# kcroker/Gadget-2.0.7-ngravs

Measured on AMD Instinct MI355X. Metric: particle-steps/s (tree+PM), higher is better.
Workload: dtype f64

## Files before the change

gadget-2.0.7-ngravs_amd/csrc/capi.hip:

```cpp
#include "engine.hpp"
#include "../../include/ngravs_peano.h"
#include <chrono>
#include <cmath>

static thread_local std::string g_create_error;

void ngravs_report(ngravs_ctx *ctx, int code, const std::string &msg)
{
  if(ctx)
    ctx->last_error = msg;
  else
    g_create_error = msg;
  if(ctx && ctx->on_fatal)
    ctx->on_fatal(code, msg.c_str());
  else
    fprintf(stderr, "task %d: endrun called with an error level of %d (%s)\n", ctx ? ctx->cfg.rank : 0, code, msg.c_str());
}

__global__ void k_pack_strided_f64(const unsigned char *src, long long stride, int ncomp, long long n, double *dst)
{
  long long i = blockIdx.x * (long long)blockDim.x + threadIdx.x;
  if(i >= n)
    return;
  const double *s = reinterpret_cast<const double *>(src + i * stride);
// ... 51 lines not shown
{
  long long k = blockIdx.x * (long long)blockDim.x + threadIdx.x;
  if(k >= count)
    return;
  const long long i = first + k;
  if(act[i] & 1)
    cost[idx[i]] = (double)nint[i];
}
__global__ void k_fill_f64(double *p, long long n, double v)
{
  long long i = blockIdx.x * (long long)blockDim.x + threadIdx.x;
  if(i < n)
    p[i] = v;
}
__global__ void k_fill_u8(unsigned char *p, long long n, unsigned char v)
{
  long long i = blockIdx.x * (long long)blockDim.x + threadIdx.x;
  if(i < n)
    p[i] = v;
}
__global__ void k_unpermute_f64(const unsigned int *idx, long long n, int ncomp, const double *src, double *dst)
{
  long long i = blockIdx.x * (long long)blockDim.x + threadIdx.x;
  if(i >= n)
    return;
  long long j = idx[i];
  for(int k = 0; k < ncomp; k++)
    dst[j * ncomp + k] = src[i * ncomp + k];
}
__global__ void k_unpermute_i2f(const unsigned int *idx, long long n, const int *src, float *dst)
{
  long long i = blockIdx.x * (long long)blockDim.x + threadIdx.x;
  if(i < n)
    dst[idx[i]] = (float)src[i];
}
__global__ void k_permute_f64(const unsigned int *idx, long long n, int ncomp, const double *src, double *dst)
{
  long long i = blockIdx.x * (long long)blockDim.x + threadIdx.x;
  if(i >= n)
    return;
  long long j = idx[i];
  for(int k = 0; k < ncomp; k++)
    dst[i * ncomp + k] = src[j * ncomp + k];
}
__global__ void k_permute_f64_lim(const unsigned int *idx, long long n, long long lim, int ncomp, const double *src, double *dst)
{
  long long i = blockIdx.x * (long long)blockDim.x + threadIdx.x;
  if(i >= n)
    return;
  long long j = idx[i];
  for(int k = 0; k < ncomp; k++)
    dst[i * ncomp + k] = j < lim ? src[j * ncomp + k] : 0.0;
}
__global__ void k_unpermute_f64_lim(const unsigned int *idx, long long n, long long lim, int ncomp, const double *src, double *dst)
{
  long long i = blockIdx.x * (long long)blockDim.x + threadIdx.x;
  if(i >= n)
    return;
  long long j = idx[i];
  if(j < lim)
    for(int k = 0; k < ncomp; k++)
      dst[j * ncomp + k] = src[i * ncomp + k];
}
__global__ void k_key18(const unsigned long long *k21, long long n, long long *out)
{
  long long i = blockIdx.x * (long long)blockDim.x + threadIdx.x;
  if(i < n)
    out[i] = (long long)(k21[i] >> (3 * (TREE_BITS - NGRAVS_BITS_PER_DIMENSION)));
}
__global__ void k_inverse_perm(const unsigned int *idx, long long n, int *inv)
{
  long long i = blockIdx.x * (long long)blockDim.x + threadIdx.x;
  if(i < n)
    inv[idx[i]] = (int)i;
}
__global__ void k_map_idx(const int *inv, const int *in, long long n, int *out)
{
  long long i = blockIdx.x * (long long)blockDim.x + threadIdx.x;
  if(i < n)
    out[i] = inv[in[i]];
}
#define GRID1(n) dim3((unsigned)(((n) + 255) / 256)), dim3(256)

extern "C" int ngravs_abi_version(void) { return NGRAVS_ABI_VERSION; }

extern "C" const char *ngravs_build_info(void)
{
  static char buf[512];
  snprintf(buf, sizeof(buf),
           "libngravs_hip abi=%d arch=gfx950 N_GRAVS<=%d NTAB=%d TREE_BITS=%d sizeof(config)=%zu sizeof(particles)=%zu "
           "sizeof(stats)=%zu walks=strict,group laws=none,newtonian,neg_newtonian,yukawa,coloyuk,bambam,sourcebambaryon,sourcebaryonbam",
           NGRAVS_ABI_VERSION, NGRAVS_MAX_GRAVS, NGRAVS_NTAB, NGRAVS_TREE_BITS, sizeof(ngravs_config_t),
           sizeof(ngravs_particles_t), sizeof(ngravs_stats_t));
  return buf;
}

extern "C" void ngravs_config_default(ngravs_config_t *cfg)
{
  memset(cfg, 0, sizeof(*cfg));
  cfg->abi_version = NGRAVS_ABI_VERSION;
  cfg->n_gravs = 1;
  cfg->G = 1.0;
  cfg->err_tol_theta = 0.5;
  cfg->err_tol_force_acc = 0.005;
  cfg->yukawa_imass = 60.0;
  cfg->tree_alloc_factor = 0.8;
  cfg->world_size = 1;
  for(int i = 0; i < NGRAVS_MAX_GRAVS; i++)
    for(int j = 0; j < NGRAVS_MAX_GRAVS; j++)
      {
        cfg->law_accel[i][j] = cfg->law_greens[i][j] = cfg->law_normed[i][j] = NGRAVS_LAW_NEWTON;
        cfg->law_spline[i][j] = NGRAVS_SPLINE_PLUMMER;
      }
}

static int check_config(const ngravs_config_t *cfg, std::string &why)
{
  if(cfg->abi_version != NGRAVS_ABI_VERSION)
    {
      why = "abi_version mismatch";
      return NGRAVS_ERR_ARG;
    }
  if(cfg->n_gravs < 1 || cfg->n_gravs > NGRAVS_MAX_GRAVS)
    {
      why = "n_gravs out of range";
      return NGRAVS_ERR_ARG;
    }
  if(cfg->pmgrid < 0 || (cfg->pmgrid & 1))
    {
      why = "PMGRID must be 0 (no mesh) or positive and even: the in-place real-to-complex mesh is laid out [N][N][N+2], which is the "
            "padding of the transform only for even N";
      return NGRAVS_ERR_ARG;
    }
  if(cfg->pmgrid && !cfg->periodic)
    {
      why = "non-periodic PM is disabled by ngravs itself (ngravs_core.c:235-242)";
      return NGRAVS_ERR_ARG;
    }
  if((cfg->periodic || cfg->pmgrid) && !(cfg->box_size > 0))
    {
      why = "box_size must be > 0";
      return NGRAVS_ERR_ARG;
    }
  if(cfg->pmgrid && cfg->type_to_grav[0] != 0)
    {
      why = "gas must be gravitational species 0 with PMGRID (ngravs_core.c:255-261)";
      return NGRAVS_ERR_WIRING;
    }
  if(cfg->world_size < 1 || cfg->rank < 0 || cfg->rank >= cfg->world_size)
    {
      why = "rank/world_size";
      return NGRAVS_ERR_ARG;
    }
  for(int t = 0; t < NGRAVS_NTYPES; t++)
    if(cfg->type_to_grav[t] < 0 || cfg->type_to_grav[t] >= cfg->n_gravs)
      {
        why = "TypeToGrav entry outside [0,N_GRAVS)";
        return NGRAVS_ERR_WIRING;
      }
  for(int i = 0; i < cfg->n_gravs; i++)
    for(int j = 0; j < cfg->n_gravs; j++)
      {
        auto bad = [](int id, int count) { return id < 0 || (id >= count && id < NGRAVS_LAW_USER0); };
        if(bad(cfg->law_accel[i][j], NGRAVS_LAW_COUNT) || bad(cfg->law_spline[i][j], NGRAVS_SPLINE_COUNT) ||
           bad(cfg->law_greens[i][j], NGRAVS_LAW_COUNT) || bad(cfg->law_normed[i][j], NGRAVS_LAW_COUNT))
          {
            why = "force-law table slot not wired (ngravs_core.c:321-360)";
            return NGRAVS_ERR_WIRING;
          }
        auto same = [](int a, int b, int p, int q) {
          return a == b || (a == p && b == q) || (a == q && b == p) || a >= NGRAVS_LAW_USER0 || b >= NGRAVS_LAW_USER0;
        };
        if(!same(cfg->law_accel[i][j], cfg->law_accel[j][i], NGRAVS_LAW_SOURCEBAM, NGRAVS_LAW_TARGETBAM) ||
           !same(cfg->law_spline[i][j], cfg->law_spline[j][i], NGRAVS_SPLINE_SOURCEBAM, NGRAVS_SPLINE_TARGETBAM) ||
           !same(cfg->law_normed[i][j], cfg->law_normed[j][i], -1, -1) || !same(cfg->law_greens[i][j], cfg->law_greens[j][i], -1, -1))
          {
            why = "force-law table violates Newton's third law (ngravs_core.c:371-403)";
            return NGRAVS_ERR_WIRING;
          }
      }
  if(cfg_has_bam(*cfg) && (cfg->pmgrid || cfg->periodic))
    {
      why = "the BAM laws have no Green's functions: tree-only, non-periodic runs (ngravs.c:189-194)";
      return NGRAVS_ERR_WIRING;
    }
  return NGRAVS_OK;
}

extern "C" int ngravs_create(const ngravs_config_t *cfg, ngravs_ctx **out) { return ngravs_create_with_laws(cfg, nullptr, 0, out); }

extern "C" int ngravs_create_with_laws(const ngravs_config_t *cfg, const ngravs_user_fn_t *fns, int nfns, ngravs_ctx **out)
{
  return ngravs_create_with_lattice(cfg, fns, nfns, nullptr, 0, out);
}

extern "C" int ngravs_create_with_lattice(const ngravs_config_t *cfg, const ngravs_user_fn_t *fns, int nfns,
                                          const ngravs_user_lattice_t *lat, int nlat, ngravs_ctx **out)
{
  if(!cfg || !out)
    return NGRAVS_ERR_ARG;
  *out = nullptr;
  std::string why;
  int rc = check_config(cfg, why);
  if(rc == NGRAVS_OK)
    rc = user_check_config(cfg, fns, nfns, lat, nlat, why);
  if(rc != NGRAVS_OK)
    {
      ngravs_report(nullptr, rc, why);
      return rc;
    }
  int ndev = 0;
  if(hipGetDeviceCount(&ndev) != hipSuccess || ndev <= 0)
    {
      ngravs_report(nullptr, NGRAVS_ERR_NO_DEVICE, "no HIP device: libngravs_hip has no CPU fallback");
      return NGRAVS_ERR_NO_DEVICE;
    }
  if(cfg->device < 0 || cfg->device >= ndev)
    return NGRAVS_ERR_ARG;
  ngravs_ctx *c = new ngravs_ctx;
  c->cfg = *cfg;
  c->user_fns.assign(fns, fns + nfns);
  c->user_lat.assign(lat, lat + nlat);
  memset(&c->stats, 0, sizeof(c->stats));
  if(hipSetDevice(cfg->device) != hipSuccess || hipStreamCreate(&c->stream) != hipSuccess ||
     hipEventCreate(&c->ev0) != hipSuccess || hipEventCreate(&c->ev1) != hipSuccess ||
     hipEventCreate(&c->evk0) != hipSuccess || hipEventCreate(&c->evk1) != hipSuccess || hipEventCreate(&c->ev_fork) != hipSuccess ||
     hipEventCreate(&c->ev_pm0) != hipSuccess || hipEventCreate(&c->ev_pm1) != hipSuccess || hipEventCreate(&c->ev_walk) != hipSuccess)
    {
      delete c;
      return NGRAVS_ERR_NO_DEVICE;
    }
  if(cfg->pmgrid)
    {
      c->asmth = cfg_asmth(cfg);
      c->rcut = cfg_rcut(cfg);
    }
  *out = c;
  return NGRAVS_OK;
}

extern "C" void ngravs_destroy(ngravs_ctx *c)
{
  if(!c)
    return;
  (void)hipSetDevice(c->cfg.device);
  (void)hipStreamSynchronize(c->stream);
  pm_release(c);
  pmslab_release(c);
  c->in_cost.release();
  c->in_pos.release();
  c->in_mass.release();
  c->in_oldacc.release();
  c->in_gsoft.release();
  c->gsoft_stage.release();
  c->s_soft.release();
  c->n_maxsoft.release();
  c->in_type.release();
  c->in_active.release();
  c->in_key.release();
  c->in_rec.release();
  c->in_id.release();
  c->dd_mask.release();
  c->dd_counts.release();
  c->dd_send.release();
  c->dd_recv.release();
  c->top.child.release();
  c->top.leaf.release();
  c->top.gcnt.release();
  c->top.info.release();
  c->top.gsum.release();
  c->top.leaf_owner.release();
  c->top.reqmask.release();
  c->top.leaf_sums.release();
  ngravs_host_toptree_free(&c->top.h);
  c->n_top.release();
  c->s_pm.release();
  c->s_type.release();
  c->s_active.release();
  c->s_oldacc.release();
  c->s_key.release();
  c->s_idx.release();
  c->idx_iota.release();
  c->sort_tmp.release();
  c->red_tmp.release();
  c->n_first.release();
  c->n_count.release();
  c->n_child.release();
  c->n_flags.release();
  c->n_nchild.release();
  c->n_geo.release();
  c->n_mom.release();
  c->n_npart.release();
  c->user_tab.release();
  c->user_green.release();
  c->scan_out.release();
  c->tb_count.release();
  c->scan_tmp.release();
  c->d_counters.release();
  c->d_levels.release();
  c->table.release();
  c->lat.release();
  c->walk_stack.release();
  c->walk_counters.release();
  c->walk_ovf.release();
  c->walk_tlist.release();
  c->walk_tmp.release();
  c->lvl_table.release();
  c->r_acc.release();
  c->r_pm.release();
  c->r_oldacc.release();
  c->r_nint.release();
  c->pm_rho.release();
  c->pm_phi.release();
  c->pm_force.release();
  c->pm_orig.release();
  c->out_tmp.release();
  c->out_tmpf.release();
  c->sph_vel_in.release();
  c->sph_h_in.release();
  c->sph_vel.release();
  c->sph_tlist.release();
  c->sph_tmp.release();
  c->sph_res.release();
  c->sph_row.release();
  c->sph_rounds.release();
  c->sph_counters.release();
  c->sph_col_in.release();
  c->sph_ts_in.release();
  c->sph_hsrc.release();
  c->sph_hmax.release();
  c->sph_gas_in.release();
  c->sph_ti_in.release();
  c->sph_tpos.release();
  c->sph_gmass.release();
  c->sph_gcount.release();
  c->sph_tg_in.release();
  c->sph_tg_ts.release();
  c->sph_tg_key.release();
  c->sph_tg_ord.release();
  c->sph_tg_res.release();
  (void)hipEventDestroy(c->ev0);
  (void)hipEventDestroy(c->ev1);
  (void)hipEventDestroy(c->evk0);
  (void)hipEventDestroy(c->evk1);
  for(hipEvent_t e : c->ev_batch)
    (void)hipEventDestroy(e);
  (void)hipEventDestroy(c->ev_fork);
  (void)hipEventDestroy(c->ev_pm0);
  (void)hipEventDestroy(c->ev_pm1);
  (void)hipEventDestroy(c->ev_walk);
  if(c->pm_stream)
    {
      (void)hipStreamSynchronize(c->pm_stream);
      (void)hipStreamSynchronize(c->walk_stream);
      (void)hipStreamDestroy(c->pm_stream);
      (void)hipStreamDestroy(c->walk_stream);
    }
  c->probe_out.release();
  (void)hipStreamDestroy(c->stream);
  delete c;
}

extern "C" void ngravs_set_fatal_handler(ngravs_ctx *ctx, ngravs_fatal_fn fn)
{
  if(ctx)
    ctx->on_fatal = fn;
}

extern "C" int ngravs_set_opening(ngravs_ctx *c, double theta, double errtol)
{
  if(!c)
    return NGRAVS_ERR_ARG;
  c->cfg.err_tol_theta = theta;
  c->cfg.err_tol_force_acc = errtol;
  return NGRAVS_OK;
}

extern "C" int ngravs_set_softening(ngravs_ctx *c, const double force_softening[NGRAVS_NTYPES])
{
  if(!c || !force_softening)
    return NGRAVS_ERR_ARG;
  for(int t = 0; t < NGRAVS_NTYPES; t++)
    if(!(force_softening[t] >= 0.0))
      {
        ngravs_report(c, NGRAVS_ERR_ARG, "ngravs_set_softening: negative or NaN softening length");
        return NGRAVS_ERR_ARG;
      }
  for(int t = 0; t < NGRAVS_NTYPES; t++)
    c->cfg.force_softening[t] = force_softening[t];
  c->gsoft_col_stale = c->gsoft_node_stale = true;
  return NGRAVS_OK;
}

extern "C" int ngravs_set_walk_mode(ngravs_ctx *c, int mode)
{
  if(!c || (mode != NGRAVS_WALK_STRICT && mode != NGRAVS_WALK_GROUP))
    return NGRAVS_ERR_ARG;
  c->cfg.walk_mode = mode;
  return NGRAVS_OK;
}

extern "C" int ngravs_get_config(ngravs_ctx *c, ngravs_config_t *out)
{
  if(!c || !out)
    return NGRAVS_ERR_ARG;
  *out = c->cfg;
  if(c->cfg.pmgrid)
    {
      out->asmth = c->asmth;
      out->rcut = c->rcut;
    }
  return NGRAVS_OK;
}

extern "C" int ngravs_set_tuning(ngravs_ctx *c, const char *name, double v)
{
  if(!c || !name)
    return NGRAVS_ERR_ARG;
  const std::string k(name);
  const long long iv = (long long)v;
  Tuning &t = c->tune;
  if(k == "walk_fused")
    t.walk_fused = iv != 0;
  else if(k == "walk_batch" && iv >= 0)
    t.walk_batch = iv;
  else if(k == "walk_waves" && iv >= 0 && iv <= 16)
    t.walk_waves = (int)iv;
  else if(k == "walk_lcap" && (iv == 0 || (iv >= 1024 && iv <= 65536)))
    {
      t.walk_lcap = (int)iv;
      c->walk_lcap = 0;
    }
  else if(k == "walk_root")
    t.walk_root = iv != 0;
  else if(k == "walk_compact")
    t.walk_compact = iv != 0;
  else if(k == "walk_spread" && iv >= 0 && iv <= 64 && (iv & (iv - 1)) == 0)
    t.walk_spread = (int)iv;
  else if(k == "walk_sg" && iv >= 0 && iv <= 16)
    t.walk_sg = (int)iv;
  else if(k == "walk_ring" && iv >= 0 && iv <= 1)
    t.walk_ring = (int)iv;
  else if(k == "walk_ring_k" && iv >= 0 && iv <= 8)
    t.walk_ring_k = (int)iv;
  else if(k == "walk_nleaf" && iv >= -1 && iv <= 8)
    t.walk_nleaf = (int)iv;
  else if(k == "walk_exact_reach")
    t.walk_exact_reach = iv != 0;
  else if(k == "sort_full")
    t.sort_full = iv != 0;
  else if(k == "tree_levelwise")
    t.tree_levelwise = iv != 0;
  else if(k == "dd_keep" && v >= 0 && v <= 0.25)
    t.dd_keep = v;
  else if(k == "pm_cus" && (iv == -1 || (iv >= 0 && iv <= 32 && iv % 8 == 0)))
    t.pm_cus = (int)iv;
  else if(k == "sph_verbose")
    t.sph_verbose = iv != 0;
  else
    {
      ngravs_report(c, NGRAVS_ERR_ARG, "ngravs_set_tuning: unknown name or value out of range: " + k);
      return NGRAVS_ERR_ARG;
    }
  return NGRAVS_OK;
}

extern "C" int ngravs_memcpy(ngravs_ctx *c, void *dst, const void *src, int64_t bytes, int kind)
{
  if(!c || bytes < 0 || kind < 1 || kind > 3 || (bytes > 0 && (!dst || !src)))
    return NGRAVS_ERR_ARG;
  if(bytes == 0)
    return NGRAVS_OK;
  (void)hipSetDevice(c->cfg.device);
  HIP_TRY(c, hipStreamSynchronize(c->stream));
  HIP_TRY(c, hipMemcpy(dst, src, (size_t)bytes, kind == 1 ? hipMemcpyHostToDevice : (kind == 2 ? hipMemcpyDeviceToHost : hipMemcpyDeviceToDevice)));
  return NGRAVS_OK;
}

extern "C" int ngravs_device_alloc(ngravs_ctx *c, void **ptr, int64_t bytes)
{
  if(!c || !ptr || bytes < 0)
    return NGRAVS_ERR_ARG;
  *ptr = nullptr;
  (void)hipSetDevice(c->cfg.device);
  if(hipMalloc(ptr, (size_t)(bytes > 0 ? bytes : 1)) != hipSuccess)
    return NGRAVS_ERR_NOMEM;
  return NGRAVS_OK;
}

extern "C" int ngravs_device_free(ngravs_ctx *c, void *ptr)
{
  if(!c)
    return NGRAVS_ERR_ARG;
  (void)hipSetDevice(c->cfg.device);
  if(ptr)
    (void)hipFree(ptr);
  return NGRAVS_OK;
}

static int upload_column_f64(ngravs_ctx *c, const void *src, int64_t stride, int ncomp, int64_t n, int on_device, double *dst)
{
  if(on_device)
    {
      if(stride == (int64_t)sizeof(double) * ncomp)
        HIP_TRY(c, hipMemcpyAsync(dst, src, sizeof(double) * ncomp * n, hipMemcpyDeviceToDevice, c->stream));
      else
        hipLaunchKernelGGL(k_pack_strided_f64, GRID1(n), 0, c->stream, (const unsigned char *)src, (long long)stride, ncomp,
                           (long long)n, dst);
      return NGRAVS_OK;
    }
  if(stride == (int64_t)sizeof(double) * ncomp)
    {
      HIP_TRY(c, hipMemcpyAsync(dst, src, sizeof(double) * ncomp * n, hipMemcpyHostToDevice, c->stream));
      HIP_TRY(c, hipStreamSynchronize(c->stream));
      return NGRAVS_OK;
    }
  c->host_stage.resize(sizeof(double) * ncomp * (size_t)n);
  double *h = reinterpret_cast<double *>(c->host_stage.data());
  for(int64_t i = 0; i < n; i++)
    memcpy(h + i * ncomp, (const unsigned char *)src + i * stride, sizeof(double) * ncomp);
  HIP_TRY(c, hipMemcpyAsync(dst, h, sizeof(double) * ncomp * n, hipMemcpyHostToDevice, c->stream));
  HIP_TRY(c, hipStreamSynchronize(c->stream));
  return NGRAVS_OK;
}

static double ev_ms(ngravs_ctx *c);

static int set_particles_impl(ngravs_ctx *c, const ngravs_particles_t *p, bool keep_tree)
{
  if(!c || !p || p->n < 0 || (p->n > 0 && (!p->pos || !p->mass || !p->type)))
    return NGRAVS_ERR_ARG;
  if(p->n == 0 && keep_tree)
    {
      if(!c->have_particles || c->n_local != 0)
        return NGRAVS_ERR_STATE;
      c->tree_stale = c->have_tree;
      return NGRAVS_OK;
    }
  if(p->n == 0)
    {
      (void)hipSetDevice(c->cfg.device);
      c->n = c->n_local = 0;
      c->own_order_nlocal = -1;
      c->sort_low = 35;
      c->all_active = true;
      c->walk_ia_ratio = 0;
      c->pm_solo_steps = 0, c->pm_auto_cus = -1;
      c->walk_unit_state = 4;
      c->have_particles = true;
      c->have_order = c->have_tree = c->have_pm = c->have_acc = false;
      c->gsoft_on = false;
      c->top.on = false;
      c->pm_parked = false;
      return NGRAVS_OK;
    }
  const bool keep_halo = keep_tree && c->n_local != c->n;
  if(keep_tree && (!c->have_order || !c->have_tree || p->n != c->n_local))
    {
      ngravs_report(c, NGRAVS_ERR_STATE, "ngravs_update_particles: needs a built tree over the same own particles");
      return NGRAVS_ERR_STATE;
    }
  if(p->n >= (1ll << 31) - 64)
    {
      ngravs_report(c, NGRAVS_ERR_ARG, "int particle indices (reference All.MaxPart is int): n must be < 2^31");
      return NGRAVS_ERR_ARG;
    }
  (void)hipSetDevice(c->cfg.device);
  const int64_t n = p->n;
  if(c->in_pos.ensure(3 * n) || c->in_mass.ensure(n) || c->in_oldacc.ensure(n) || c->in_type.ensure(n) || c->in_active.ensure(n) ||
     (!keep_tree && c->in_cost.ensure(n)))
    {
      ngravs_report(c, NGRAVS_ERR_NOMEM, "device allocation failed");
      return NGRAVS_ERR_NOMEM;
    }
  if(!keep_halo)
    c->n = n;
  c->n_local = n;
  if(!keep_tree)
    {
      if(c->own_order_nlocal != n)
        c->own_order_nlocal = -1;
      c->sort_low = 35;
    }
  int rc;
  if(!keep_tree && (rc = dd_fill_ids(c)))
    return rc;
  if((rc = upload_column_f64(c, p->pos, p->pos_stride, 3, n, p->on_device, c->in_pos.p)))
    return rc;
  if((rc = upload_column_f64(c, p->mass, p->mass_stride, 1, n, p->on_device, c->in_mass.p)))
    return rc;
  if(p->old_acc)
    {
      if((rc = upload_column_f64(c, p->old_acc, p->old_acc_stride, 1, n, p->on_device, c->in_oldacc.p)))
        return rc;
    }
  else
    hipLaunchKernelGGL(k_fill_f64, GRID1(n), 0, c->stream, c->in_oldacc.p, (long long)n, 0.0);
  if(!keep_tree)
    {
      if(p->grav_cost && p->on_device)
        hipLaunchKernelGGL(k_pack_strided_f32_to_f64, GRID1(n), 0, c->stream, (const unsigned char *)p->grav_cost,
                           (long long)p->grav_cost_stride, (long long)n, c->in_cost.p);
      else if(p->grav_cost)
        {
          c->host_stage.resize(sizeof(double) * (size_t)n);
          double *h = reinterpret_cast<double *>(c->host_stage.data());
// ... 240 lines not shown
      c->have_order = true;
      c->have_tree = c->tree_stale = c->have_pm = false;
      c->stats.t_domain = c->stats.t_peano = 0;
      return NGRAVS_OK;
    }
  HIP_TRY(c, hipEventRecord(c->ev0, c->stream));
  int rc = dom_find_extent(c);
  if(rc)
    return rc;
  HIP_TRY(c, hipEventRecord(c->ev1, c->stream));
  c->stats.t_domain = ev_ms(c) * 1e-3;
  HIP_TRY(c, hipEventRecord(c->ev0, c->stream));
  c->own_order_nlocal = -1;
  rc = dom_keys_and_sort(c);
  if(rc)
    return rc;
  c->own_order_nlocal = c->n_local;
  c->own_order_len = c->n;
  HIP_TRY(c, hipEventRecord(c->ev1, c->stream));
  c->stats.t_peano = ev_ms(c) * 1e-3;
  int64_t ws = c->cfg.world_size, r = c->cfg.rank;
  int64_t lo = (c->n * r) / ws, hi = (c->n * (r + 1)) / ws;
  lo = (lo / 64) * 64;
  hi = (r + 1 == ws) ? c->n : (hi / 64) * 64;
  c->shard_first = lo;
  c->shard_count = hi - lo;
  c->have_order = true;
  c->have_tree = false;
  c->gsoft_col_stale = c->gsoft_node_stale = true;
  c->tree_stale = false;
  if(c->have_pm)
    {
      if(c->r_pm.ensure(3 * c->n))
        return NGRAVS_ERR_NOMEM;
      hipLaunchKernelGGL(k_permute_f64_lim, GRID1(c->n), 0, c->stream, c->s_idx.p, (long long)c->n, (long long)c->n_local, 3, c->pm_orig.p,
                         c->r_pm.p);
      HIP_TRY(c, hipGetLastError());
    }
  return NGRAVS_OK;
}

extern "C" int ngravs_domain_decomposition(ngravs_ctx *c) { return domain_decomposition_impl(c, true); }

extern "C" int ngravs_discard_grav_pm(ngravs_ctx *c)
{
  if(!c)
    return NGRAVS_ERR_ARG;
  c->have_pm = false;
  c->pm_parked = false;
  return NGRAVS_OK;
}

extern "C" int64_t ngravs_force_treebuild(ngravs_ctx *c)
{
  if(!c || !c->have_order)
    return NGRAVS_ERR_STATE;
  (void)hipSetDevice(c->cfg.device);
  if(c->n == 0)
    {
      c->nnodes = 0;
      c->have_tree = true;
      c->tree_refit = false;
      c->stats.t_treebuild = 0;
      return 0;
    }
  if(hipEventRecord(c->ev0, c->stream) != hipSuccess)
    return NGRAVS_ERR_NO_DEVICE;
  int rc = tree_build(c);
  if(rc)
    return rc;
  if(hipEventRecord(c->ev1, c->stream) != hipSuccess)
    return NGRAVS_ERR_NO_DEVICE;
  c->stats.t_treebuild = ev_ms(c) * 1e-3;
  c->have_tree = true;
  c->tree_refit = false;
  c->gsoft_node_stale = true;
  return c->nnodes;
}

static int ensure_table(ngravs_ctx *c)
{
  if(!c->cfg.pmgrid || c->table_ready)
    return NGRAVS_OK;
  const int ng = c->cfg.n_gravs;
  std::vector<double> h((size_t)(ng * ng + 1) * NTAB);
  host_shortrange_table(&c->cfg, h.data(), nullptr, c->user_fns.data(), (int)c->user_fns.size());
  {
    WalkParams wp;
    make_walk_params(c, &wp);
    for(int t = 0; t < NTAB; t++)
      h[(size_t)ng * ng * NTAB + t] = exp(-wp.ym * (double)t * wp.inv_asmthfac);
  }
  if(c->table.ensure(h.size()))
    return NGRAVS_ERR_NOMEM;
  HIP_TRY(c, hipMemcpyAsync(c->table.p, h.data(), sizeof(double) * h.size(), hipMemcpyHostToDevice, c->stream));
  HIP_TRY(c, hipStreamSynchronize(c->stream));
  c->table_ready = true;
  return NGRAVS_OK;
}

static bool pm_cu_bit(int R, int b)
{
  const int x = b / 32, k = b - 33 * x;
  return b < 256 && k >= 0 && k % 8 == 0 && k / 8 < R / 8;
}

static int masked_streams(ngravs_ctx *c, int R)
{
  if(c->pm_stream && c->pm_stream_cus == R)
    return NGRAVS_OK;
  if(!c->device_cus)
    {
      hipDeviceProp_t prop;
      HIP_TRY(c, hipGetDeviceProperties(&prop, c->cfg.device));
      c->device_cus = prop.multiProcessorCount;
    }
  if(c->device_cus != 256 || R < 8 || R > 32 || R % 8)
    return NGRAVS_ERR_ARG;
  if(c->pm_stream)
    {
      HIP_TRY(c, hipStreamSynchronize(c->pm_stream));
      HIP_TRY(c, hipStreamSynchronize(c->walk_stream));
      (void)hipStreamDestroy(c->pm_stream);
      (void)hipStreamDestroy(c->walk_stream);
      c->pm_stream = c->walk_stream = nullptr;
      c->pm_stream_cus = 0;
    }
  uint32_t mp[8] = {0}, mw[8] = {0};
  for(int b = 0; b < 256; b++)
    (pm_cu_bit(R, b) ? mp : mw)[b / 32] |= 1u << (b % 32);
  hipStream_t sp = nullptr, sw = nullptr;
  if(hipExtStreamCreateWithCUMask(&sp, 8, mp) != hipSuccess || hipExtStreamCreateWithCUMask(&sw, 8, mw) != hipSuccess)
    {
      if(sp)
        (void)hipStreamDestroy(sp);
      (void)hipGetLastError();
      return NGRAVS_ERR_NO_DEVICE;
    }
  uint32_t gp[8] = {0}, gw[8] = {0};
  if(hipExtStreamGetCUMask(sp, 8, gp) != hipSuccess || hipExtStreamGetCUMask(sw, 8, gw) != hipSuccess || memcmp(gp, mp, sizeof mp) ||
     memcmp(gw, mw, sizeof mw))
    {
      (void)hipStreamDestroy(sp);
      (void)hipStreamDestroy(sw);
      (void)hipGetLastError();
      return NGRAVS_ERR_NO_DEVICE;
    }
  c->pm_stream = sp;
  c->walk_stream = sw;
  c->pm_stream_cus = R;
  return NGRAVS_OK;
}

static bool overlap_eligible(const ngravs_ctx *c)
{
  return c->cfg.pmgrid && c->cfg.periodic && c->cfg.world_size == 1 && !c->top.on && c->cfg.walk_mode == NGRAVS_WALK_GROUP &&
         c->n > 0 && c->n_local > 0;
}

static int gravity_tree_begin(ngravs_ctx *c, bool beside_pm, bool *masked, bool *empty)
{
  *masked = *empty = false;
  if(!c || !c->have_order)
    return NGRAVS_ERR_STATE;
  (void)hipSetDevice(c->cfg.device);
  int rc;
  if(!c->have_tree)
    {
      int64_t nn = ngravs_force_treebuild(c);
      if(nn < 0)
        return (int)nn;
    }
  else if(c->tree_stale && (rc = ngravs_force_update_tree(c)))
    return rc;
  if((rc = ensure_table(c)))
    return rc;
  if(c->n_local == 0)
    {
      c->stats.t_treewalk = 0;
      c->stats.walk_kernel_ms = 0;
      c->stats.interactions = 0;
      c->stats.n_active = 0;
      c->have_acc = true;
      *empty = true;
      return NGRAVS_OK;
    }
  HIP_TRY(c, hipEventRecord(c->ev0, c->stream));
  *masked = (beside_pm || (c->tune.pm_cus > 0 && overlap_eligible(c))) && masked_streams(c, beside_pm ? c->pm_stream_cus : c->tune.pm_cus) == NGRAVS_OK;
  if(*masked)
    {
      HIP_TRY(c, hipStreamWaitEvent(c->walk_stream, c->ev0, 0));
      OnStream on(c, c->walk_stream, c->device_cus - c->pm_stream_cus);
      return walk_enqueue(c);
    }
  return walk_enqueue(c);
}

static int gravity_tree_end(ngravs_ctx *c, bool masked, hipEvent_t pm_done)
{
  int rc;
  if(masked)
    {
      {
        OnStream on(c, c->walk_stream, c->device_cus - c->pm_stream_cus);
        if((rc = walk_complete(c)))
          return rc;
      }
      HIP_TRY(c, hipEventRecord(c->ev_walk, c->walk_stream));
      HIP_TRY(c, hipStreamWaitEvent(c->stream, c->ev_walk, 0));
    }
  else if((rc = walk_complete(c)))
    return rc;
  if(pm_done)
    HIP_TRY(c, hipStreamWaitEvent(c->stream, pm_done, 0));
  if((rc = walk_finish(c)))
    return rc;
  HIP_TRY(c, hipEventRecord(c->ev1, c->stream));
  c->stats.t_treewalk = ev_ms(c) * 1e-3;
  float kms = 0;
  (void)hipEventSynchronize(c->evk1);
  (void)hipEventElapsedTime(&kms, c->evk0, c->evk1);
  c->stats.walk_kernel_ms = kms;
  double h[2] = {0, 0};
  HIP_TRY(c, hipMemcpyAsync(h, c->red_tmp.p, 2 * sizeof(double), hipMemcpyDeviceToHost, c->stream));
  HIP_TRY(c, hipStreamSynchronize(c->stream));
  c->stats.interactions = h[0];
  c->stats.n_active = (int64_t)h[1];
  c->have_acc = true;
  if(c->cfg.pmgrid && c->cfg.walk_mode == NGRAVS_WALK_GROUP && h[1] > 0 && c->cfg.box_size > 0)
    {
      const double reach = (c->cfg.group_reach > 0 ? c->cfg.group_reach : NGRAVS_GROUP_REACH) * c->asmth;
      const double ntot = c->top.on && c->top.total_count > 0 ? c->top.total_count : (double)c->n;
      const double L = c->cfg.box_size, expect = 4.18879020478639 * reach * reach * reach * ntot / (L * L * L);
      const bool dense = c->walk_ntargets < 0 || c->walk_dense_tlist;
      if(expect > 0 && dense)
        {
          const double f_sg = c->walk_sg >= 4 ? 1.0 : (c->walk_sg >= 2 ? 1857.0 / 1393.0 : 1857.0 / 1079.0);
          const double f_s = c->walk_spread >= 2 ? 1079.0 / 871.0 : 1.0;
          c->walk_ia_ratio = (h[0] / h[1]) / expect * f_sg * f_s;
        }
    }
  if(c->shard_count > 0 && c->extent_override)
    hipLaunchKernelGGL(k_cost_update, GRID1(c->shard_count), 0, c->stream, c->s_idx.p, c->s_active.p, c->r_nint.p,
                       (long long)c->shard_first, (long long)c->shard_count, c->in_cost.p);
  return NGRAVS_OK;
}

extern "C" int ngravs_gravity_tree(ngravs_ctx *c)
{
  bool masked, empty;
  const int rc = gravity_tree_begin(c, false, &masked, &empty);
  return (rc || empty) ? rc : gravity_tree_end(c, masked, nullptr);
}

static int pm_on_masked_stream(ngravs_ctx *c)
{
  HIP_TRY(c, hipEventRecord(c->ev_fork, c->stream));
  HIP_TRY(c, hipStreamWaitEvent(c->pm_stream, c->ev_fork, 0));
  OnStream on(c, c->pm_stream, c->pm_stream_cus);
  HIP_TRY(c, hipEventRecord(c->ev_pm0, c->stream));
  int rc = pm_run(c);
  if(rc)
    return rc;
  HIP_TRY(c, hipEventRecord(c->ev_pm1, c->stream));
  return NGRAVS_OK;
}

extern "C" int ngravs_pmforce_periodic(ngravs_ctx *c)
{
  if(!c || !c->have_particles)
    return NGRAVS_ERR_STATE;
  (void)hipSetDevice(c->cfg.device);
  int rc;
  if(!c->have_order && (rc = ngravs_domain_decomposition(c)))
    return rc;
  if(!c->have_tree)
    {
      int64_t nn = ngravs_force_treebuild(c);
      if(nn < 0)
        return (int)nn;
    }
  else if(c->tree_stale && (rc = ngravs_force_update_tree(c)))
    return rc;
  if(c->tune.pm_cus > 0 && overlap_eligible(c) && masked_streams(c, c->tune.pm_cus) == NGRAVS_OK)
    {
      if((rc = pm_on_masked_stream(c)))
        return rc;
      float ms = 0;
      HIP_TRY(c, hipEventSynchronize(c->ev_pm1));
      (void)hipEventElapsedTime(&ms, c->ev_pm0, c->ev_pm1);
      HIP_TRY(c, hipStreamWaitEvent(c->stream, c->ev_pm1, 0));
      c->stats.t_pm = ms * 1e-3;
      return NGRAVS_OK;
    }
  HIP_TRY(c, hipEventRecord(c->ev0, c->stream));
  if((rc = pm_run(c)))
    return rc;
  HIP_TRY(c, hipEventRecord(c->ev1, c->stream));
  c->stats.t_pm = ev_ms(c) * 1e-3;
  return NGRAVS_OK;
}

static const double PM_CU_SCALE[4] = {17.75, 9.07, 6.16, 4.74};
static const double PM_FIT_MARGIN = 1.05, PM_SHARE_COST = 1.04;
static int choose_pm_cus(ngravs_ctx *c)
{
  if(!overlap_eligible(c))
    return 0;
  if(c->tune.pm_cus >= 0)
    return c->tune.pm_cus;
  if(c->pm_auto_cus >= 0)
    return c->pm_auto_cus;
  if(c->pm_solo_steps < 2 || c->pm_solo_ms <= 0 || c->walk_solo_ms <= 0)
    return 0;
  c->pm_auto_cus = 0;
  for(int m = 1; m <= 4; m++)
    {
      const double walk = c->walk_solo_ms * 256.0 / (256 - 8 * m);
      if(c->pm_solo_ms * PM_CU_SCALE[m - 1] * PM_FIT_MARGIN < walk)
        {
          if(walk * PM_SHARE_COST < 0.99 * (c->pm_solo_ms + c->walk_solo_ms))
            c->pm_auto_cus = 8 * m;
          break;
        }
    }
  return c->pm_auto_cus;
}

extern "C" int ngravs_compute_accelerations(ngravs_ctx *c, int pm_step)
{
  if(!c || !c->have_particles)
    return NGRAVS_ERR_STATE;
  int rc;
  if((rc = domain_decomposition_impl(c, !(pm_step && c->cfg.pmgrid))))
    return rc;
  c->last_pm_cus = 0;
  if(!(pm_step && c->cfg.pmgrid))
    return ngravs_gravity_tree(c);
  const int R = choose_pm_cus(c);
  if(R > 0 && masked_streams(c, R) == NGRAVS_OK)
    {
      int64_t nn = ngravs_force_treebuild(c);
      if(nn < 0)
        return (int)nn;
      bool masked, empty;
      if((rc = gravity_tree_begin(c, true, &masked, &empty)))
        return rc;
      if((rc = pm_on_masked_stream(c)))
        return rc;
      if(!empty && (rc = gravity_tree_end(c, masked, c->ev_pm1)))
        return rc;
      float ms = 0;
      (void)hipEventElapsedTime(&ms, c->ev_pm0, c->ev_pm1);
      c->stats.t_pm = ms * 1e-3;
      c->last_pm_cus = R;
      if(c->tune.pm_cus < 0 && ms > c->stats.walk_kernel_ms)
        c->pm_auto_cus = R < 32 ? R + 8 : 0;
      return NGRAVS_OK;
    }
  if((rc = ngravs_pmforce_periodic(c)))
    return rc;
  if((rc = ngravs_gravity_tree(c)))
    return rc;
  if(overlap_eligible(c) && c->tune.pm_cus < 0 && c->pm_auto_cus < 0)
    {
      c->pm_solo_ms = c->stats.t_pm * 1e3;
      c->walk_solo_ms = c->stats.walk_kernel_ms;
      c->pm_solo_steps++;
    }
  return NGRAVS_OK;
}

static int download_strided(ngravs_ctx *c, const void *dsrc, size_t elem, int ncomp, int64_t n, void *dst, int64_t stride,
                            int on_device)
{
  const size_t row = elem * ncomp;
  if(on_device)
    {
      if((size_t)stride != row)
        {
          ngravs_report(c, NGRAVS_ERR_ARG, "device outputs must be contiguous");
          return NGRAVS_ERR_ARG;
        }
      HIP_TRY(c, hipMemcpyAsync(dst, dsrc, row * n, hipMemcpyDeviceToDevice, c->stream));
      HIP_TRY(c, hipStreamSynchronize(c->stream));
      return NGRAVS_OK;
    }
  if((size_t)stride == row)
    {
      HIP_TRY(c, hipMemcpyAsync(dst, dsrc, row * n, hipMemcpyDeviceToHost, c->stream));
      HIP_TRY(c, hipStreamSynchronize(c->stream));
      return NGRAVS_OK;
    }
  c->host_stage.resize(row * (size_t)n);
  HIP_TRY(c, hipMemcpyAsync(c->host_stage.data(), dsrc, row * n, hipMemcpyDeviceToHost, c->stream));
  HIP_TRY(c, hipStreamSynchronize(c->stream));
  for(int64_t i = 0; i < n; i++)
    memcpy((unsigned char *)dst + i * stride, c->host_stage.data() + i * row, row);
  return NGRAVS_OK;
}

static int deliver(ngravs_ctx *c, const void *dsrc, size_t elem, int ncomp, int64_t n, void *dst, int64_t stride, int on_device,
                   const unsigned char *d_mask)
{
  if(!d_mask)
    return download_strided(c, dsrc, elem, ncomp, n, dst, stride, on_device);
  const size_t row = elem * ncomp;
  if(on_device)
    {
      if((size_t)stride != row)
        {
          ngravs_report(c, NGRAVS_ERR_ARG, "device outputs must be contiguous");
          return NGRAVS_ERR_ARG;
        }
      if(elem == sizeof(double))
        hipLaunchKernelGGL(k_copy_masked_f64, GRID1(n), 0, c->stream, d_mask, (long long)n, ncomp, (const double *)dsrc, (double *)dst);
      else
        hipLaunchKernelGGL(k_copy_masked_f32, GRID1(n), 0, c->stream, d_mask, (long long)n, (const float *)dsrc, (float *)dst);
      HIP_TRY(c, hipStreamSynchronize(c->stream));
      return NGRAVS_OK;
    }
  c->host_stage.resize(row * (size_t)n + (size_t)n);
  unsigned char *hm = c->host_stage.data() + row * (size_t)n;
  HIP_TRY(c, hipMemcpyAsync(c->host_stage.data(), dsrc, row * n, hipMemcpyDeviceToHost, c->stream));
  HIP_TRY(c, hipMemcpyAsync(hm, d_mask, (size_t)n, hipMemcpyDeviceToHost, c->stream));
  HIP_TRY(c, hipStreamSynchronize(c->stream));
  for(int64_t i = 0; i < n; i++)
    if(hm[i] & 1)
      memcpy((unsigned char *)dst + i * stride, c->host_stage.data() + i * row, row);
  return NGRAVS_OK;
}

extern "C" int ngravs_get_accel(ngravs_ctx *c, double *grav_accel, int64_t accel_stride, double *grav_pm, int64_t pm_stride,
                                double *old_acc, int64_t old_acc_stride, float *grav_cost, int64_t cost_stride, int on_device,
                                int only_active)
{
  if(!c || !c->have_order)
    return NGRAVS_ERR_STATE;
  (void)hipSetDevice(c->cfg.device);
  const int64_t n = c->n, nl = c->n_local;
  if(nl == 0)
    return NGRAVS_OK;
  if(c->out_tmp.ensure(3 * n) || c->out_tmpf.ensure(n))
    return NGRAVS_ERR_NOMEM;
  const unsigned char *mask = only_active ? c->in_active.p : nullptr;
  int rc;
  if(grav_accel)
    {
      if(!c->have_acc)
        return NGRAVS_ERR_STATE;
      HIP_TRY(c, hipMemsetAsync(c->out_tmp.p, 0, sizeof(double) * 3 * n, c->stream));
      hipLaunchKernelGGL(k_unpermute_f64, GRID1(n), 0, c->stream, c->s_idx.p, (long long)n, 3, c->r_acc.p, c->out_tmp.p);
      if((rc = deliver(c, c->out_tmp.p, sizeof(double), 3, nl, grav_accel, accel_stride, on_device, mask)))
        return rc;
    }
  if(grav_pm)
    {
      if(!c->have_pm)
        return NGRAVS_ERR_STATE;
      hipLaunchKernelGGL(k_unpermute_f64, GRID1(n), 0, c->stream, c->s_idx.p, (long long)n, 3, c->r_pm.p, c->out_tmp.p);
      if((rc = deliver(c, c->out_tmp.p, sizeof(double), 3, nl, grav_pm, pm_stride, on_device, nullptr)))
        return rc;
    }
  if(old_acc)
    {
      if(!c->have_acc)
        return NGRAVS_ERR_STATE;
      hipLaunchKernelGGL(k_unpermute_f64, GRID1(n), 0, c->stream, c->s_idx.p, (long long)n, 1, c->r_oldacc.p, c->out_tmp.p);
      if((rc = deliver(c, c->out_tmp.p, sizeof(double), 1, nl, old_acc, old_acc_stride, on_device, mask)))
        return rc;
    }
  if(grav_cost)
    {
      if(!c->have_acc)
        return NGRAVS_ERR_STATE;
      hipLaunchKernelGGL(k_unpermute_i2f, GRID1(n), 0, c->stream, c->s_idx.p, (long long)n, c->r_nint.p, c->out_tmpf.p);
      if((rc = deliver(c, c->out_tmpf.p, sizeof(float), 1, nl, grav_cost, cost_stride, on_device, mask)))
        return rc;
    }
  return NGRAVS_OK;
}

extern "C" int ngravs_get_stats(ngravs_ctx *c, ngravs_stats_t *out)
{
  if(!c || !out)
    return NGRAVS_ERR_ARG;
  *out = c->stats;
  return NGRAVS_OK;
}

static std::string kept_state(const ngravs_ctx *c, const char *who)
{
  char b[320];
  snprintf(b, sizeof(b), "%s: no kept decomposition to work on (own rows %lld, rows at the cut %lld, working set %lld, tree %d, top %d, task %d of %d)", who,
           (long long)c->n_local, (long long)c->top.own_leaf_n, (long long)c->n, (int)c->have_tree, (int)c->top.on, c->top.kept_rank, c->top.kept_world);
  return std::string(b);
}
extern "C" int ngravs_dd_leaf_sums_kept(ngravs_ctx *c, void **dev_sums, int64_t *count)
{
  if(!c || !dev_sums || !count)
    return NGRAVS_ERR_ARG;
  (void)hipSetDevice(c->cfg.device);
  const int rc = dd_leaf_sums_kept(c, dev_sums, count);
  if(rc == NGRAVS_ERR_STATE)
    ngravs_report(c, rc, kept_state(c, "ngravs_dd_leaf_sums_kept"));
  return rc;
}
extern "C" int ngravs_dd_pack_leaves_kept(ngravs_ctx *c, int64_t *counts, void **dev_records, int64_t *nrec)
{
  if(!c || !counts || !dev_records || !nrec)
    return NGRAVS_ERR_ARG;
  (void)hipSetDevice(c->cfg.device);
  const int rc = dd_pack_leaves_kept(c, counts, dev_records, nrec);
  if(rc == NGRAVS_ERR_STATE)
    ngravs_report(c, rc, kept_state(c, "ngravs_dd_pack_leaves_kept"));
  return rc;
}
extern "C" int ngravs_dd_refresh_halo(ngravs_ctx *c, const void *dev_records, int64_t nrec)
{
  if(!c || nrec < 0 || (nrec > 0 && !dev_records))
    return NGRAVS_ERR_ARG;
  (void)hipSetDevice(c->cfg.device);
  const int rc = dd_refresh_halo(c, dev_records, nrec);
  if(rc == NGRAVS_ERR_STATE)
    ngravs_report(c, rc, kept_state(c, "ngravs_dd_refresh_halo"));
  return rc;
}
extern "C" int ngravs_dd_update_top(ngravs_ctx *c, const double *node_sums, const double *leaf_len)
{
  if(!c)
    return NGRAVS_ERR_ARG;
  (void)hipSetDevice(c->cfg.device);
  const int rc = dd_update_top(c, node_sums, leaf_len);
  if(rc == NGRAVS_ERR_STATE)
    ngravs_report(c, rc, kept_state(c, "ngravs_dd_update_top"));
  return rc;
}
extern "C" int ngravs_dd_get_kept(ngravs_ctx *c, int32_t *rank, int32_t *world, const int32_t **leaf_owner, const uint8_t **present,
                                  const double **node_sums)
{
  if(!c)
    return NGRAVS_ERR_ARG;
  const TopTree &t = c->top;
  if(!(t.on && t.h.nnode > 0 && t.own_leaf_n == c->n_local && t.kept_rank >= 0 && (int)t.h_leaf_owner.size() == t.h.nleaf &&
       (int)t.h_present.size() == t.h.nleaf))
    {
      ngravs_report(c, NGRAVS_ERR_STATE, kept_state(c, "ngravs_dd_get_kept"));
      return NGRAVS_ERR_STATE;
    }
  if(rank)
    *rank = t.kept_rank;
  if(world)
    *world = t.kept_world;
  if(leaf_owner)
    *leaf_owner = t.h_leaf_owner.data();
  if(present)
    *present = t.h_present.data();
  if(node_sums)
    *node_sums = t.h_node_sums.data();
  return NGRAVS_OK;
}

extern "C" int ngravs_walk_unopened(ngravs_ctx *c, int64_t *count)
{
  if(!c || !count)
    return NGRAVS_ERR_ARG;
  *count = (int64_t)c->walk_unopened;
  return NGRAVS_OK;
}

extern "C" int ngravs_get_domain(ngravs_ctx *c, double out[8])
{
  if(!c || !c->have_order)
    return NGRAVS_ERR_STATE;
  memcpy(out, c->dom, sizeof(double) * 8);
  return NGRAVS_OK;
}

extern "C" int ngravs_get_keys(ngravs_ctx *c, int64_t *keys, int on_device)
{
  if(!c || !c->have_order || !keys)
    return NGRAVS_ERR_STATE;
  (void)hipSetDevice(c->cfg.device);
  const int64_t n = c->n;
  if(c->out_tmp.ensure(3 * n))
    return NGRAVS_ERR_NOMEM;
  long long *tmp = reinterpret_cast<long long *>(c->out_tmp.p);
  hipLaunchKernelGGL(k_key18, GRID1(n), 0, c->stream, c->in_key.p, (long long)n, tmp);
  return download_strided(c, tmp, sizeof(long long), 1, c->n_local, keys, sizeof(long long), on_device);
}

extern "C" int ngravs_get_order(ngravs_ctx *c, int32_t *order, int on_device)
{
  if(!c || !c->have_order || !order)
    return NGRAVS_ERR_STATE;
  (void)hipSetDevice(c->cfg.device);
  return download_strided(c, c->s_idx.p, sizeof(int), 1, c->n, order, sizeof(int), on_device);
}

extern "C" int ngravs_get_shard(ngravs_ctx *c, int64_t *first, int64_t *count)
{
  if(!c || !c->have_order)
    return NGRAVS_ERR_STATE;
  if(first)
    *first = c->shard_first;
  if(count)
    *count = c->shard_count;
// ... 959 lines not shown
```

gadget-2.0.7-ngravs_amd/csrc/engine.hpp:

```cpp
#pragma once
#include <hip/hip_runtime.h>
#include <cstdint>
#include <cstdio>
#include <cstdlib>
#include <cstring>
#include <string>
#include <utility>
#include <vector>
#include "../../include/ngravs_host.h"

#define NG_MAX NGRAVS_MAX_GRAVS
#define NTAB NGRAVS_NTAB
#define TREE_BITS NGRAVS_TREE_BITS
#define FLAG_BUCKET 64
#define FLAG_PSEUDO 128
#define FLAG_PARTIAL 256
#define FLAG_SPECIES_SHIFT 9
#define FLAG_SPECIES_SLOTS 8
#define FLAG_SPECIES_MASK (0xffff << FLAG_SPECIES_SHIFT)
#define MAX_LEVELS (TREE_BITS + 1)

struct ngravs_ctx;

#define HIP_TRY(ctx, expr)                                                                        \
  do                                                                                              \
    {                                                                                             \
      hipError_t e__ = (expr);                                                                    \
      if(e__ != hipSuccess)                                                                       \
        {                                                                                         \
          ngravs_report(ctx, NGRAVS_ERR_NO_DEVICE, std::string(#expr) + ": " + hipGetErrorString(e__)); \
          return NGRAVS_ERR_NO_DEVICE;                                                            \
        }                                                                                         \
    }                                                                                             \
  while(0)

void ngravs_report(ngravs_ctx *ctx, int code, const std::string &msg);

template <typename T> struct DevBuf
{
  T *p = nullptr;
  size_t cap = 0;
  int ensure(size_t n)
  {
    if(n <= cap)
      return 0;
    if(p)
      (void)hipFree(p);
    p = nullptr;
    cap = 0;
    size_t want = n + n / 16 + 64;
    if(hipMalloc((void **)&p, want * sizeof(T)) != hipSuccess)
      return -1;
    cap = want;
    return 0;
  }
  void release()
  {
    if(p)
      (void)hipFree(p);
    p = nullptr;
    cap = 0;
  }
};

#define UL_NC 8
struct UserTabs
{
  const double *coef, *spl;
  int e_lo, n_oct, S;
  int nh, Ss;
  double h[NGRAVS_NTYPES];
};
__host__ __device__ inline double ul_poly(const double *c, double t)
{
  double v = c[7];
  for(int j = 6; j >= 0; j--)
    v = v * t + c[j];
  return v;
}
__host__ __device__ inline double ul_g(const UserTabs &u, int k, double r)
{
  int e;
  (void)frexp(r, &e);
  int o = e - u.e_lo;
  const double m = ldexp(r, -(u.e_lo + (o < 0 ? 0 : (o >= u.n_oct ? u.n_oct - 1 : o))));
  double s = (m - 0.5) * (2 * u.S);
  s = o < 0 ? 0.0 : (o >= u.n_oct ? (double)u.S : s);
  o = o < 0 ? 0 : (o >= u.n_oct ? u.n_oct - 1 : o);
  s = s >= 0 ? (s <= u.S ? s : (double)u.S) : 0.0;
  int j = (int)s;
  j = j >= u.S ? u.S - 1 : j;
  return ul_poly(u.coef + ((size_t)(k * u.n_oct + o) * u.S + j) * UL_NC, 2 * (s - j) - 1);
}
__host__ __device__ inline double ul_spline(const UserTabs &u, int k, double h, double r)
{
  if(u.nh == 0)
    return 0.0;
  int i = 0;
  for(int q = 1; q < u.nh; q++)
    if(fabs(u.h[q] - h) < fabs(u.h[i] - h))
      i = q;
  double s = r / h * u.Ss;
  s = s >= 0 ? (s <= u.Ss ? s : (double)u.Ss) : 0.0;
  int j = (int)s;
  j = j >= u.Ss ? u.Ss - 1 : j;
  return ul_poly(u.spl + ((size_t)(k * u.nh + i) * u.Ss + j) * UL_NC, 2 * (s - j) - 1);
}

struct WalkParams
{
  int ng, periodic, pm, use_theta;
  int nleaf;
  int exact_reach;
  double box, boxhalf;
  double theta2;
  double errtol_acc;
  double rcut, rcut2, asmthfac, utor2wpi, reach2;
  double ym;
  double bam_eps;
  double fac_intp;
  double fsoft[NGRAVS_NTYPES];
  int t2g[NGRAVS_NTYPES];
  unsigned t2g_packed;
  double cN[NG_MAX][NG_MAX], cY[NG_MAX][NG_MAX], cS[NG_MAX][NG_MAX];
  int ntab_lds;
  int tab_slot[NG_MAX * NG_MAX];
  int slot_src[NG_MAX * NG_MAX];
  int exp_tab;
  double inv_asmthfac;
  double ec[4];
  int src_in_box;
  int bam;
  int law_accel[NG_MAX][NG_MAX], law_spline[NG_MAX][NG_MAX];
  int user;
  UserTabs ut;
};

struct TreeView
{
  const int *first, *count, *child, *flags;
  const int *npart;
  const double4 *geo, *mom;
  int nnodes;
  const int *ltab;
  int ltab_level;
  double ltab_corner[3], ltab_cl;
  const double *soft;
  const double *maxsoft;
};

struct Tuning
{
  int walk_fused = 0, walk_waves = 0, walk_lcap = 0, walk_root = 0, walk_compact = 1, walk_spread = 0, walk_exact_reach = 0, walk_sg = 0, walk_nleaf = -1;
  long long walk_batch = 0;
  int sort_full = 0;
  int tree_levelwise = 0;
  double dd_keep = 0;
  int walk_ring = 1;
  int walk_ring_k = 0;
  int pm_cus = -1;
  int sph_verbose = 0;
};

#define TOP_CW(ng) (7 + 4 * (ng))
struct TopTree
{
  double total_count = 0;
  bool on = false;
  double import_reach = 0;
  ngravs_toptree h = {0, 0, 0, 0, nullptr, nullptr, nullptr, nullptr, nullptr};
  DevBuf<int> child, leaf;
  DevBuf<int> gcnt;
  DevBuf<unsigned char> info;
  DevBuf<double> gsum;
  DevBuf<int> leaf_owner;
  DevBuf<unsigned long long> reqmask;
  DevBuf<double> leaf_sums;
  DevBuf<int> own_leaf;
  long long own_leaf_n = -1;
  int kept_rank = -1, kept_world = 0;
  std::vector<int> h_leaf_owner;
  std::vector<unsigned char> h_present;
  std::vector<double> h_node_sums;
  DevBuf<int> kept_row;
  std::vector<int64_t> kept_counts;
  long long kept_total = -1;
  DevBuf<double> kept_sums;
  DevBuf<double> leaf_len;
};

struct PmSlab
{
  int world = 0, rank = 0, N = 0, stage = -1;
  int xs = 0, nx = 0, ys = 0, ny = 0;
  int lo[3] = {0, 0, 0}, ext[3] = {0, 0, 0};
  int elo[3] = {0, 0, 0}, eext[3] = {0, 0, 0};
  std::vector<int> bbox;
  std::vector<int64_t> scount, rcount;
  long long edesc_off = 0;
  DevBuf<double> brick, slab, tbuf, ebrick, fmesh, send, recv;
  DevBuf<long long> desc;
  std::vector<long long> hdesc[2];
  int hdesc_turn = 0;
  void *plan2f = nullptr, *plan2i = nullptr, *plan1 = nullptr;
  int plan_N = 0, plan_nx = 0, plan_ny = 0;
  double bytes_sent[4] = {0, 0, 0, 0};
};

struct ngravs_ctx
{
  ngravs_config_t cfg;
  Tuning tune;
  PmSlab pms;
  TopTree top;
  DevBuf<int> n_top;
  ngravs_fatal_fn on_fatal = nullptr;
  hipStream_t stream = nullptr;
  double asmth = 0, rcut = 0;
  int64_t n = 0;
  int64_t n_local = 0;
  bool extent_override = false;
  double ext_lo[3], ext_hi[3];
  int dd_last_what = -1;
  long long dd_last_sent = 0;
  bool have_particles = false, have_order = false, have_tree = false, have_pm = false, have_acc = false;
  bool pm_parked = false;
  double dom[8] = {0, 0, 0, 0, 0, 0, 0, 0};
  double pos_lo[3] = {0, 0, 0}, pos_hi[3] = {-1, -1, -1};
  int64_t shard_first = 0, shard_count = 0;

  DevBuf<double> in_pos, in_mass, in_oldacc;
  DevBuf<double> in_cost;
  DevBuf<int> in_type;
  DevBuf<unsigned char> in_active;
  DevBuf<double2> in_rec;
  DevBuf<unsigned long long> in_key;
  DevBuf<long long> in_id;
  DevBuf<unsigned long long> dd_mask, dd_counts;
  int sort_low = 35;
  long long own_order_nlocal = -1, own_order_len = 0;
  DevBuf<unsigned char> dd_send, dd_recv;
  DevBuf<double4> s_pm;
  DevBuf<unsigned char> s_type, s_active;
  DevBuf<double> s_oldacc;
  DevBuf<unsigned long long> s_key;
  DevBuf<unsigned int> s_idx, idx_iota;
  DevBuf<unsigned char> sort_tmp;
  DevBuf<double> red_tmp;
  int64_t max_nodes = 0, nnodes = 0;
  bool tree_refit = false;
  bool tree_stale = false;
  int nlevels = 0;
  DevBuf<int> lvl_table;
  int lvl_table_level = 0;
  int64_t level_start[MAX_LEVELS + 2];
  DevBuf<int> n_first, n_count, n_child, n_flags, n_nchild;
  DevBuf<double4> n_geo, n_mom;
  DevBuf<int> tb_count;
  DevBuf<int> n_npart;
  DevBuf<int> scan_out;
  DevBuf<unsigned char> scan_tmp;
  DevBuf<int> d_counters;
  DevBuf<int> d_levels;
  long long level_hint[MAX_LEVELS + 2] = {0};
  DevBuf<double> table;
  bool table_ready = false;
  DevBuf<double> lat;
  bool lat_ready = false;
  DevBuf<int> walk_stack;
  DevBuf<int> walk_tlist;
  DevBuf<unsigned char> walk_tmp;
  long long walk_ntargets = -1;
  bool walk_dense_tlist = false;
  int walk_spread = 0;
  int walk_sg = 1;
  long long walk_unopened = 0;
  int walk_unit_state = 4;
  double walk_ia_ratio = 0;
  bool all_active = true;
  DevBuf<int> walk_ovf;
  DevBuf<int> walk_counters;
  DevBuf<double> r_acc, r_pm, r_oldacc;
  DevBuf<int> r_nint;
  int pm_plan_n = 0;
  void *fft_fwd = nullptr, *fft_inv = nullptr;
  DevBuf<double> pm_rho;
  DevBuf<double> pm_force;
  DevBuf<double> pm_phi;
  DevBuf<double> pm_orig;
  DevBuf<double> out_tmp;
  DevBuf<float> out_tmpf;
  std::vector<unsigned char> host_stage;
  ngravs_stats_t stats;
  hipEvent_t ev0 = nullptr, ev1 = nullptr, evk0 = nullptr, evk1 = nullptr;
  std::vector<hipEvent_t> ev_batch;
  int walk_batches = 0;
  int walk_lcap = 0;
  int walk_scap = 0;
  bool walk_used_split = false;
  long long walk_cap_n = -1;
  size_t walk_cap_stack = 0;
  size_t walk_cap_bytes = 0;
  std::vector<std::pair<const void *, size_t>> walk_lds_set;
  std::string last_error;
  std::vector<ngravs_user_fn_t> user_fns;
  std::vector<ngravs_user_lattice_t> user_lat;
  DevBuf<double> user_tab;
  UserTabs user_ut = {};
  bool user_ready = false;
  double user_soft[NGRAVS_NTYPES] = {0, 0, 0, 0, 0, 0};
  int last_walk_kernel = 0;
  bool gsoft_on = false;
  bool gsoft_col_stale = true, gsoft_node_stale = true;
  DevBuf<double> in_gsoft;
  DevBuf<double> gsoft_stage;
  DevBuf<double> s_soft;
  DevBuf<double> n_maxsoft;
  hipStream_t pm_stream = nullptr, walk_stream = nullptr;
  int pm_stream_cus = 0;
  int device_cus = 0;
  int stream_cus = 0;
  int last_pm_cus = 0;
  double pm_solo_ms = 0, walk_solo_ms = 0;
  int pm_solo_steps = 0;
  int pm_auto_cus = -1;
  hipEvent_t ev_fork = nullptr, ev_pm0 = nullptr, ev_pm1 = nullptr, ev_walk = nullptr;
  DevBuf<int> probe_out;
  DevBuf<double> user_green;
  long long user_green_nk2 = 0;
  DevBuf<double> sph_vel_in, sph_h_in;
  DevBuf<double> sph_vel;
  DevBuf<int> sph_tlist;
  DevBuf<unsigned char> sph_tmp;
  DevBuf<double> sph_res;
  DevBuf<int> sph_row, sph_rounds;
  DevBuf<unsigned long long> sph_counters;
  DevBuf<double> sph_col_in;
  DevBuf<int> sph_ts_in;
  DevBuf<double> sph_hsrc;
  DevBuf<double> sph_hmax;
  DevBuf<double> sph_gas_in;
  DevBuf<int> sph_ti_in;
  DevBuf<int> sph_tpos;
  DevBuf<double> sph_gmass;
  DevBuf<int> sph_gcount;
  DevBuf<double> sph_tg_in;
  DevBuf<int> sph_tg_ts;
  DevBuf<unsigned long long> sph_tg_key;
  DevBuf<unsigned int> sph_tg_ord;
  DevBuf<double> sph_tg_res;
};

struct OnStream
{
  ngravs_ctx *c;
  hipStream_t s0;
  int n0;
  OnStream(ngravs_ctx *c_, hipStream_t s, int cus) : c(c_), s0(c_->stream), n0(c_->stream_cus)
  {
    c->stream = s;
    c->stream_cus = cus;
  }
  ~OnStream()
  {
    c->stream = s0;
    c->stream_cus = n0;
  }
};

int dom_find_extent(ngravs_ctx *c);
int dom_keys_and_sort(ngravs_ctx *c);
int dom_keys_only(ngravs_ctx *c, const double *d_pos, int64_t n, const double corner[3], double fac, int bits,
                  long long *d_keys);
int dd_local_extent(ngravs_ctx *c, double lo[3], double hi[3]);
void dd_apply_extent(ngravs_ctx *c, const double lo[3], const double hi[3]);
int dd_set_toptree(ngravs_ctx *c, int nnode, const int *child);
int dd_leaf_sums(ngravs_ctx *c, void **dev_sums, int64_t *count);
int dd_pack(ngravs_ctx *c, int what, const int *leaf_owner, int nranks, int me, int64_t *counts, void **dev_records, int64_t *nrec);
int dd_apply_migration(ngravs_ctx *c, const void *dev_records, int64_t nrec);
int dd_get_dest(ngravs_ctx *c, const int *leaf_owner, int *dest);
int dd_target_bounds(ngravs_ctx *c, double out[2]);
int dd_pack_leaves(ngravs_ctx *c, const unsigned long long *reqmask, int nranks, int me, int64_t *counts, void **dev_records, int64_t *nrec);
int dd_set_top(ngravs_ctx *c, const double *node_sums, const unsigned char *present);
int dd_set_halo(ngravs_ctx *c, const void *dev_records, int64_t nrec);
int dd_leaf_sums_kept(ngravs_ctx *c, void **dev_sums, int64_t *count);
int dd_pack_leaves_kept(ngravs_ctx *c, int64_t *counts, void **dev_records, int64_t *nrec);
int dd_refresh_halo(ngravs_ctx *c, const void *dev_records, int64_t nrec);
int dd_update_top(ngravs_ctx *c, const double *node_sums, const double *leaf_len);
int dd_peano_order_own(ngravs_ctx *c, int force);
int dd_fill_ids(ngravs_ctx *c);
int dd_record_doubles(const ngravs_ctx *c, int what);
int tree_build(ngravs_ctx *c);
int tree_moments(ngravs_ctx *c, bool refit, bool counts = false);
int tree_top_leaf_len(ngravs_ctx *c, double *dev_kept_sums, int stride);
int tree_top_refit(ngravs_ctx *c);
int dom_regather(ngravs_ctx *c);
static inline bool cfg_has_bam(const ngravs_config_t &cfg)
{
  for(int i = 0; i < cfg.n_gravs; i++)
    for(int j = 0; j < cfg.n_gravs; j++)
      if((cfg.law_accel[i][j] >= NGRAVS_LAW_BAMBAM && cfg.law_accel[i][j] < NGRAVS_LAW_USER0) ||
         (cfg.law_spline[i][j] >= NGRAVS_SPLINE_BAMBAM && cfg.law_spline[i][j] < NGRAVS_SPLINE_USER0))
        return true;
  return false;
}
static inline bool cfg_has_user(const ngravs_config_t &cfg)
{
  for(int i = 0; i < cfg.n_gravs; i++)
    for(int j = 0; j < cfg.n_gravs; j++)
      if(cfg.law_accel[i][j] >= NGRAVS_LAW_USER0 || cfg.law_spline[i][j] >= NGRAVS_SPLINE_USER0)
        return true;
  return false;
}
int user_check_config(const ngravs_config_t *cfg, const ngravs_user_fn_t *fns, int nfns, const ngravs_user_lattice_t *lat, int nlat,
                      std::string &why);
ngravs_lattice_fn user_lattice_fn(const ngravs_ctx *c, int a, int b);
bool user_lattice_complete(const ngravs_ctx *c);
int user_lattice_tabulate(ngravs_lattice_fn fn, double box, double *out, std::string &why);
void ngravs_report(ngravs_ctx *ctx, int code, const std::string &msg);
int user_tables_ensure(ngravs_ctx *c, double r_need);
int user_green_ensure(ngravs_ctx *c);
double user_normed(const ngravs_user_fn_t *fns, int nfns, int law, double k2);
void make_walk_params(const ngravs_ctx *c, WalkParams *wp);
int walk_run(ngravs_ctx *c);
int walk_enqueue(ngravs_ctx *c);
int walk_complete(ngravs_ctx *c);
int walk_finish(ngravs_ctx *c);
int direct_run(ngravs_ctx *c, const int *d_idx, int64_t nt, double *d_acc);
int direct_run_targets(ngravs_ctx *c, const double4 *d_tpm, const int *d_ttype, int64_t nt, double *d_acc, double r_need = 0);
int adaptive_refresh(ngravs_ctx *c, bool nodes);
int eval_ring_slots(const WalkParams &wp, bool yuk, int waves);
int launch_eval_ring(ngravs_ctx *c, const TreeView &tv, const WalkParams &wp, bool yuk, int nblk, int waves, int K, const int *region,
                     const int *gcount, long long g0, long long nb, int lcap, int scap, int S, const int *tlist, int SG, long long t_count);
#define SPH_KC1 2.546479089470
#define SPH_KC2 15.278874536822
#define SPH_KC3 45.836623610466
#define SPH_KC4 30.557749073644
#define SPH_KC5 5.092958178941
#define SPH_KC6 (-15.278874536822)
#define SPH_NORM_COEFF 4.188790204786
#define SPH_MAXITER 150
__host__ __device__ inline void sph_spline(double u, double hinv3, double hinv4, double *wk, double *dwk)
{
  if(u < 0.5)
    {
      *wk = hinv3 * (SPH_KC1 + SPH_KC2 * (u - 1) * u * u);
      *dwk = hinv4 * u * (SPH_KC3 * u - SPH_KC4);
    }
  else
    {
      *wk = hinv3 * SPH_KC5 * (1.0 - u) * (1.0 - u) * (1.0 - u);
      *dwk = hinv4 * SPH_KC6 * (1.0 - u) * (1.0 - u);
    }
}
enum { SPH_HSML = 0, SPH_DENSITY, SPH_NUMNGB, SPH_DIVVEL, SPH_CURLVEL, SPH_DHSML, SPH_NRES };
struct SphStats
{
  long long targets, bad_hsml, failed, stack_ovf, max_rounds, sum_rounds, candidates, neighbours;
};
int sph_density_run(ngravs_ctx *c, double des_num_ngb, double max_dev, double min_hsml, SphStats *st);
int sph_hsml_guess_run(ngravs_ctx *c, double des_num_ngb, int only_unset, long long *rows, long long *bad_mass);
enum { SPH_HS_VX = 0, SPH_HS_VY, SPH_HS_VZ, SPH_HS_H, SPH_HS_RHO, SPH_HS_POR2, SPH_HS_CSJ, SPH_HS_F2, SPH_HS_TS, SPH_HS_CSI, SPH_HS_F1,
       SPH_HS_NCOL };
enum { SPH_HY_ACCX = 0, SPH_HY_ACCY, SPH_HY_ACCZ, SPH_HY_DTENTR, SPH_HY_MAXSIG, SPH_HY_NRES };
struct SphHydroParams
{
  int periodic, comoving, limiter, have_ts;
  double box, boxhalf;
  double hubble_a2, fac_mu, fac_vsic_fix;
  double visc, tbi, gamma;
};
struct SphHydroStats
{
  long long targets, bad_hsml, bad_density, bad_pressure, stack_ovf, candidates, pairs;
};
int sph_hydro_run(ngravs_ctx *c, const SphHydroParams &hp, SphHydroStats *st);
enum { SPH_GAS_PRESSURE = SPH_NRES, SPH_GAS_HYDRO, SPH_GAS_NRES = SPH_GAS_HYDRO + SPH_HY_NRES };
struct SphGasParams
{
  double des, dev, minh;
  int ti_current, have_dte;
};
int sph_gas_run(ngravs_ctx *c, const SphGasParams &gp, const SphHydroParams &hp, SphStats *ds, SphHydroStats *hs, hipEvent_t ev_density,
                hipEvent_t ev_prep);
struct SphScatterCols
{
  unsigned char *dst[SPH_GAS_NRES];
  long long stride[SPH_GAS_NRES];
};
int sph_scatter_cols(ngravs_ctx *c, long long nt, const SphScatterCols &cols);
int sph_scatter(ngravs_ctx *c, const double *src, long long nt, double *dst, long long stride);
enum { SPH_SUM_RHO = 0, SPH_SUM_NGB, SPH_SUM_DHR, SPH_SUM_DIV, SPH_SUM_ROTX, SPH_SUM_ROTY, SPH_SUM_ROTZ, SPH_NSUMS };
enum { SPH_TG_H = 6, SPH_TG_MASS, SPH_TG_RHO, SPH_TG_P, SPH_TG_DHSML, SPH_TG_F1, SPH_TG_NCOL };
struct SphSumsStats
{
  long long bad_hsml, bad_density, bad_pressure, bad_pos, stack_ovf, candidates, pairs;
};
int sph_density_sums_run(ngravs_ctx *c, long long nt, SphSumsStats *st);
int sph_hydro_sums_run(ngravs_ctx *c, const SphHydroParams &hp, long long nt, int have_tts, SphSumsStats *st, SphHydroStats *own);
__host__ __device__ inline int sph_density_update_one(const double *s, double des, double dev, double minh, double *h_io, double *left_io,
                                                      double *right_io, int *rounds_io, double *out6)
{
#pragma clang fp contract(off)
  double h = *h_io, left = *left_io, right = *right_io;
  const int nr = ++*rounds_io;
  const double numngb = s[SPH_SUM_NGB], rho = s[SPH_SUM_RHO];
  const double dhf = 1 / (1 + h * s[SPH_SUM_DHR] / (3 * rho));
  bool redo = numngb < (des - dev) || (numngb > (des + dev) && h > 1.01 * minh);
  if(redo && left > 0 && right > 0 && (right - left) < 1.0e-3 * left)
    redo = false;
  if(!redo)
    {
      out6[SPH_HSML] = h;
      out6[SPH_DENSITY] = rho;
      out6[SPH_NUMNGB] = numngb;
      out6[SPH_DIVVEL] = s[SPH_SUM_DIV] / rho;
      out6[SPH_CURLVEL] = sqrt(s[SPH_SUM_ROTX] * s[SPH_SUM_ROTX] + s[SPH_SUM_ROTY] * s[SPH_SUM_ROTY] + s[SPH_SUM_ROTZ] * s[SPH_SUM_ROTZ]) / rho;
      out6[SPH_DHSML] = dhf;
      return 0;
    }
  if(numngb < (des - dev))
    left = fmax(h, left);
  else if(right != 0)
    {
      if(h < right)
        right = h;
    }
  else
    right = h;
  if(right > 0 && left > 0)
    h = pow(0.5 * (pow(left, 3) + pow(right, 3)), 1.0 / 3);
  else
    {
      const bool newton = fabs(numngb - des) < 0.5 * des;
      const double fac = 1 - (numngb - des) / (3 * numngb) * dhf;
      if(right == 0 && left > 0)
        h *= newton ? fac : 1.26;
      if(right > 0 && left == 0)
        h = newton ? h * fac : h / 1.26;
    }
  if(h < minh)
    h = minh;
  *h_io = h, *left_io = left, *right_io = right;
  return nr > SPH_MAXITER ? 2 : 1;
}
int sph_density_update_device(long long n, const double *sums, double *h, double *left, double *right, int *rounds, double des, double dev,
                              double minh, int *accepted, double *const out[SPH_NRES], long long *failed);
int pm_run(ngravs_ctx *c);
int pm_deposit(ngravs_ctx *c);
int pm_finish(ngravs_ctx *c);
void pm_release(ngravs_ctx *c);
int pmslab_begin(ngravs_ctx *c, int rank, int world, int bbox[6]);
int pmslab_pack(ngravs_ctx *c, int stage, const int *all_bbox, int64_t *send_counts, int64_t *recv_counts, void **send, void **recv);
int pmslab_unpack(ngravs_ctx *c, int stage);
void pmslab_release(ngravs_ctx *c);
void host_shortrange_table(const ngravs_config_t *cfg, double *force, double *pot, const ngravs_user_fn_t *fns = nullptr, int nfns = 0);
double cfg_asmth(const ngravs_config_t *c);
double cfg_rcut(const ngravs_config_t *c);
```

gadget-2.0.7-ngravs_amd/csrc/eval_asm.inc:

```


#define ER_FST_OFF_ET "16640"
#define ER_FST_OFF_NOET "256"

#define ER_YUK_ET \
  "v_fract_f64_e32 v[118:119], v[118:119]\n"                                   \
  "v_mul_f64 v[122:123], v[118:119], %[ec3]\n" \
  "v_lshl_add_u32 v113, v112, 3, %[etab]\n" \
  "v_add_f64 v[122:123], v[122:123], -%[ec2]\n" \
  "ds_read_b64 v[124:125], v113\n"                                             \
  "v_lshl_add_u32 v112, v112, 3, %[trow]\n" \
  "v_fma_f64 v[122:123], v[122:123], v[118:119], %[ec1]\n" \
  "ds_read_b64 v[112:113], v112\n"                                             \
  "v_fma_f64 v[122:123], v[122:123], v[118:119], -%[ec0]\n" \
  "v_mul_f64 v[120:121], v[114:115], v[114:115]\n"                             \
  "v_fma_f64 v[122:123], v[122:123], v[118:119], 1.0\n"                        \
  "s_waitcnt lgkmcnt(1)\n" \
  "v_mul_f64 v[122:123], v[124:125], v[122:123]\n"                             \
  "v_mul_f64 v[122:123], %[cY], v[122:123]\n" \
  "v_fma_f64 v[124:125], %[ym], v[114:115], v[120:121]\n"                      \
  "v_mul_f64 v[122:123], v[124:125], v[122:123]\n" \
  "v_fmac_f64_e32 v[122:123], %[cN], v[120:121]\n"

#define ER_NOYUK \
  "v_lshl_add_u32 v112, v112, 3, %[trow]\n" \
  "ds_read_b64 v[112:113], v112\n" \
  "v_mul_f64 v[120:121], v[114:115], v[114:115]\n" \
  "v_mul_f64 v[122:123], %[cN], v[120:121]\n"

#define ER_DIRECT_ASM \
  "s_mov_b32 s89, 0\n" \
  "ds_read_b128 v[104:107], %[ptr]\n" \
  "ds_read_b128 v[108:111], %[ptr] offset:16\n" \
  "s_bitcmp1_b32 %[n], 0\n"                                                    \
  "s_cbranch_scc0 L_ed_pairs_%=\n" \
  "s_waitcnt lgkmcnt(0)\n" \
  "v_add_f64 v[104:105], v[104:105], -%[tpx]\n" \
  "v_add_f64 v[106:107], v[106:107], -%[tpy]\n" \
  "v_mul_f64 v[112:113], v[106:107], v[106:107]\n" \
  "v_add_f64 v[108:109], v[108:109], -%[tpz]\n" \
  "v_fmac_f64_e32 v[112:113], v[104:105], v[104:105]\n" \
  "v_fmac_f64_e32 v[112:113], v[108:109], v[108:109]\n" \
  "v_add_f64 v[116:117], v[112:113], %[tiny]\n"                                \
  "v_rsq_f64_e32 v[114:115], v[116:117]\n" \
  "v_cmp_gt_f64_e32 vcc, %[h2max], v[112:113]\n"                               \
  "v_mul_f64 v[118:119], v[116:117], v[114:115]\n"                             \
  "v_fma_f64 v[118:119], -v[118:119], v[114:115], 1.0\n" \
  "v_mul_f64 v[120:121], v[114:115], 0.5\n" \
  "v_fma_f64 v[114:115], v[120:121], v[118:119], v[114:115]\n"                 \
  "v_mul_f64 v[120:121], v[114:115], v[114:115]\n" \
  "v_mul_f64 v[122:123], %[cN], v[120:121]\n"                                  \
  "v_mul_f64 v[122:123], v[110:111], v[122:123]\n" \
  "v_mul_f64 v[122:123], v[114:115], v[122:123]\n"                             \
  "s_cbranch_vccnz L_ed_softs_%=\n" \
  "L_ed_accs_%=:\n" \
  "v_fmac_f64_e32 %[ax], v[104:105], v[122:123]\n" \
  "v_fmac_f64_e32 %[ay], v[106:107], v[122:123]\n" \
  "v_fmac_f64_e32 %[az], v[108:109], v[122:123]\n" \
  "s_mov_b32 s89, 1\n" \
  "v_add_u32_e32 %[ptr], 32, %[ptr]\n" \
  "ds_read_b128 v[104:107], %[ptr]\n"                                          \
  "ds_read_b128 v[108:111], %[ptr] offset:16\n" \
  "L_ed_pairs_%=:\n" \
  "s_cmp_lt_u32 s89, %[n]\n" \
  "s_cbranch_scc0 L_ed_done_%=\n" \
  "L_ed_topx_%=:\n" \
  "s_waitcnt lgkmcnt(0)\n" \
  "ds_read_b128 v[96:99], %[ptr] offset:32\n" \
  "ds_read_b128 v[100:103], %[ptr] offset:48\n" \
  "v_add_f64 v[104:105], v[104:105], -%[tpx]\n" \
  "v_add_f64 v[106:107], v[106:107], -%[tpy]\n" \
  "v_mul_f64 v[112:113], v[106:107], v[106:107]\n" \
  "v_add_f64 v[108:109], v[108:109], -%[tpz]\n" \
  "v_fmac_f64_e32 v[112:113], v[104:105], v[104:105]\n" \
  "v_fmac_f64_e32 v[112:113], v[108:109], v[108:109]\n" \
  "v_add_f64 v[116:117], v[112:113], %[tiny]\n"                                \
  "v_rsq_f64_e32 v[114:115], v[116:117]\n" \
  "v_cmp_gt_f64_e32 vcc, %[h2max], v[112:113]\n"                               \
  "v_mul_f64 v[118:119], v[116:117], v[114:115]\n"                             \
  "v_fma_f64 v[118:119], -v[118:119], v[114:115], 1.0\n" \
  "v_mul_f64 v[120:121], v[114:115], 0.5\n" \
  "v_fma_f64 v[114:115], v[120:121], v[118:119], v[114:115]\n"                 \
  "v_mul_f64 v[120:121], v[114:115], v[114:115]\n" \
  "v_mul_f64 v[122:123], %[cN], v[120:121]\n"                                  \
  "v_mul_f64 v[122:123], v[110:111], v[122:123]\n" \
  "v_mul_f64 v[122:123], v[114:115], v[122:123]\n"                             \
  "s_cbranch_vccnz L_ed_softx_%=\n" \
  "L_ed_accx_%=:\n" \
  "v_fmac_f64_e32 %[ax], v[104:105], v[122:123]\n" \
  "v_fmac_f64_e32 %[ay], v[106:107], v[122:123]\n" \
  "v_fmac_f64_e32 %[az], v[108:109], v[122:123]\n" \
  "s_waitcnt lgkmcnt(0)\n" \
  "v_add_u32_e32 %[ptr], 64, %[ptr]\n" \
  "ds_read_b128 v[104:107], %[ptr]\n"                                          \
  "ds_read_b128 v[108:111], %[ptr] offset:16\n" \
  "v_add_f64 v[96:97], v[96:97], -%[tpx]\n" \
  "v_add_f64 v[98:99], v[98:99], -%[tpy]\n" \
  "v_mul_f64 v[112:113], v[98:99], v[98:99]\n" \
  "v_add_f64 v[100:101], v[100:101], -%[tpz]\n" \
  "v_fmac_f64_e32 v[112:113], v[96:97], v[96:97]\n" \
  "v_fmac_f64_e32 v[112:113], v[100:101], v[100:101]\n" \
  "v_add_f64 v[116:117], v[112:113], %[tiny]\n"                                \
  "v_rsq_f64_e32 v[114:115], v[116:117]\n" \
  "v_cmp_gt_f64_e32 vcc, %[h2max], v[112:113]\n"                               \
  "v_mul_f64 v[118:119], v[116:117], v[114:115]\n"                             \
  "v_fma_f64 v[118:119], -v[118:119], v[114:115], 1.0\n" \
  "v_mul_f64 v[120:121], v[114:115], 0.5\n" \
  "v_fma_f64 v[114:115], v[120:121], v[118:119], v[114:115]\n"                 \
  "v_mul_f64 v[120:121], v[114:115], v[114:115]\n" \
  "v_mul_f64 v[122:123], %[cN], v[120:121]\n"                                  \
  "v_mul_f64 v[122:123], v[102:103], v[122:123]\n" \
  "v_mul_f64 v[122:123], v[114:115], v[122:123]\n"                             \
  "s_cbranch_vccnz L_ed_softy_%=\n" \
  "L_ed_accy_%=:\n" \
  "v_fmac_f64_e32 %[ax], v[96:97], v[122:123]\n" \
  "v_fmac_f64_e32 %[ay], v[98:99], v[122:123]\n" \
  "v_fmac_f64_e32 %[az], v[100:101], v[122:123]\n" \
  "s_add_u32 s89, s89, 2\n" \
  "s_cmp_lt_u32 s89, %[n]\n" \
  "s_cbranch_scc1 L_ed_topx_%=\n" \
  "s_branch L_ed_done_%=\n" \
  "L_ed_softs_%=:\n" \
  "v_mul_f64 v[116:117], v[116:117], v[114:115]\n"                             \
  "v_add_u32_e32 v118, s89, %[tyb]\n"                                          \
  "ds_read_u8 v118, v118\n" \
  "s_waitcnt lgkmcnt(0)\n" \
  "v_lshl_add_u32 v118, v118, 3, %[fst]\n" \
  "ds_read_b64 v[124:125], v118\n"                                             \
  "s_waitcnt lgkmcnt(0)\n" \
  "v_max_f64 v[124:125], v[124:125], %[hT]\n"                                  \
  "v_rcp_f64_e32 v[112:113], v[124:125]\n" \
  "v_cmp_lt_f64_e64 s[94:95], v[116:117], v[124:125]\n"                        \
  "v_fma_f64 v[118:119], -v[124:125], v[112:113], 1.0\n"                       \
  "v_fma_f64 v[112:113], v[112:113], v[118:119], v[112:113]\n" \
  "v_fma_f64 v[118:119], -v[124:125], v[112:113], 1.0\n" \
  "v_fma_f64 v[112:113], v[112:113], v[118:119], v[112:113]\n"                 \
  "v_mul_f64 v[114:115], v[124:125], v[114:115]\n"                             \
  "v_mul_f64 v[118:119], v[116:117], v[112:113]\n"                             \
  "v_mul_f64 v[120:121], v[118:119], v[118:119]\n"                             \
  "v_ldexp_f64 v[124:125], v[118:119], 5\n"                                    \
  "s_mov_b32 s90, 0x33333333\n" \
  "s_mov_b32 s91, 0x40433333\n" \
  "v_add_f64 v[124:125], v[124:125], -s[90:91]\n" \
  "s_mov_b32 s92, 0x55555611\n" \
  "s_mov_b32 s93, 0x40255555\n" \
  "v_fma_f64 v[124:125], v[120:121], v[124:125], s[92:93]\n"                   \
  "v_mul_f64 v[116:117], v[120:121], v[118:119]\n"                             \
  "v_mul_f64 v[120:121], v[120:121], s[90:91]\n"                               \
  "s_mov_b32 s90, 0x555554f8\n" \
  "s_mov_b32 s91, 0x40355555\n" \
  "v_add_f64 v[120:121], v[120:121], s[90:91]\n"                               \
  "s_mov_b32 s90, 0x00000000\n" \
  "s_mov_b32 s91, 0xc0480000\n" \
  "v_fma_f64 v[120:121], v[118:119], s[90:91], v[120:121]\n"                   \
  "v_fma_f64 v[120:121], -v[116:117], s[92:93], v[120:121]\n"                  \
  "v_mul_f64 v[116:117], v[114:115], v[114:115]\n" \
  "v_mul_f64 v[116:117], v[116:117], v[114:115]\n"                             \
  "s_mov_b32 s90, 0x11116ee4\n" \
  "s_mov_b32 s91, 0x3fb11111\n" \
  "v_fma_f64 v[120:121], -v[116:117], s[90:91], v[120:121]\n"                  \
  "v_cmp_gt_f64_e32 vcc, 0.5, v[118:119]\n"                                    \
  "v_cndmask_b32_e32 v120, v120, v124, vcc\n" \
  "v_cndmask_b32_e32 v121, v121, v125, vcc\n" \
  "v_mul_f64 v[124:125], %[cS], v[110:111]\n"                                  \
  "v_mul_f64 v[124:125], v[124:125], v[112:113]\n" \
  "v_mul_f64 v[124:125], v[124:125], v[112:113]\n" \
  "v_mul_f64 v[124:125], v[124:125], v[112:113]\n" \
  "v_mul_f64 v[124:125], v[124:125], v[120:121]\n" \
  "v_cndmask_b32_e64 v122, v122, v124, s[94:95]\n" \
  "v_cndmask_b32_e64 v123, v123, v125, s[94:95]\n" \
  "s_branch L_ed_accs_%=\n" \
  "L_ed_softx_%=:\n" \
  "v_mul_f64 v[116:117], v[116:117], v[114:115]\n"                             \
  "v_add_u32_e32 v118, s89, %[tyb]\n"                                          \
  "ds_read_u8 v118, v118\n" \
  "s_waitcnt lgkmcnt(0)\n" \
  "v_lshl_add_u32 v118, v118, 3, %[fst]\n" \
  "ds_read_b64 v[124:125], v118\n"                                             \
  "s_waitcnt lgkmcnt(0)\n" \
  "v_max_f64 v[124:125], v[124:125], %[hT]\n"                                  \
  "v_rcp_f64_e32 v[112:113], v[124:125]\n" \
  "v_cmp_lt_f64_e64 s[94:95], v[116:117], v[124:125]\n"                        \
  "v_fma_f64 v[118:119], -v[124:125], v[112:113], 1.0\n"                       \
  "v_fma_f64 v[112:113], v[112:113], v[118:119], v[112:113]\n" \
  "v_fma_f64 v[118:119], -v[124:125], v[112:113], 1.0\n" \
  "v_fma_f64 v[112:113], v[112:113], v[118:119], v[112:113]\n"                 \
  "v_mul_f64 v[114:115], v[124:125], v[114:115]\n"                             \
  "v_mul_f64 v[118:119], v[116:117], v[112:113]\n"                             \
  "v_mul_f64 v[120:121], v[118:119], v[118:119]\n"                             \
  "v_ldexp_f64 v[124:125], v[118:119], 5\n"                                    \
  "s_mov_b32 s90, 0x33333333\n" \
  "s_mov_b32 s91, 0x40433333\n" \
  "v_add_f64 v[124:125], v[124:125], -s[90:91]\n" \
  "s_mov_b32 s92, 0x55555611\n" \
  "s_mov_b32 s93, 0x40255555\n" \
  "v_fma_f64 v[124:125], v[120:121], v[124:125], s[92:93]\n"                   \
  "v_mul_f64 v[116:117], v[120:121], v[118:119]\n"                             \
  "v_mul_f64 v[120:121], v[120:121], s[90:91]\n"                               \
  "s_mov_b32 s90, 0x555554f8\n" \
  "s_mov_b32 s91, 0x40355555\n" \
  "v_add_f64 v[120:121], v[120:121], s[90:91]\n"                               \
  "s_mov_b32 s90, 0x00000000\n" \
  "s_mov_b32 s91, 0xc0480000\n" \
  "v_fma_f64 v[120:121], v[118:119], s[90:91], v[120:121]\n"                   \
  "v_fma_f64 v[120:121], -v[116:117], s[92:93], v[120:121]\n"                  \
  "v_mul_f64 v[116:117], v[114:115], v[114:115]\n" \
  "v_mul_f64 v[116:117], v[116:117], v[114:115]\n"                             \
  "s_mov_b32 s90, 0x11116ee4\n" \
  "s_mov_b32 s91, 0x3fb11111\n" \
  "v_fma_f64 v[120:121], -v[116:117], s[90:91], v[120:121]\n"                  \
  "v_cmp_gt_f64_e32 vcc, 0.5, v[118:119]\n"                                    \
  "v_cndmask_b32_e32 v120, v120, v124, vcc\n" \
  "v_cndmask_b32_e32 v121, v121, v125, vcc\n" \
  "v_mul_f64 v[124:125], %[cS], v[110:111]\n"                                  \
  "v_mul_f64 v[124:125], v[124:125], v[112:113]\n" \
  "v_mul_f64 v[124:125], v[124:125], v[112:113]\n" \
  "v_mul_f64 v[124:125], v[124:125], v[112:113]\n" \
  "v_mul_f64 v[124:125], v[124:125], v[120:121]\n" \
  "v_cndmask_b32_e64 v122, v122, v124, s[94:95]\n" \
  "v_cndmask_b32_e64 v123, v123, v125, s[94:95]\n" \
  "s_branch L_ed_accx_%=\n" \
  "L_ed_softy_%=:\n" \
  "v_mul_f64 v[116:117], v[116:117], v[114:115]\n"                             \
  "s_add_u32 s88, s89, 1\n" \
  "v_add_u32_e32 v118, s88, %[tyb]\n"                                          \
  "ds_read_u8 v118, v118\n" \
  "s_waitcnt lgkmcnt(0)\n" \
  "v_lshl_add_u32 v118, v118, 3, %[fst]\n" \
  "ds_read_b64 v[124:125], v118\n"                                             \
  "s_waitcnt lgkmcnt(0)\n" \
  "v_max_f64 v[124:125], v[124:125], %[hT]\n"                                  \
  "v_rcp_f64_e32 v[112:113], v[124:125]\n" \
  "v_cmp_lt_f64_e64 s[94:95], v[116:117], v[124:125]\n"                        \
  "v_fma_f64 v[118:119], -v[124:125], v[112:113], 1.0\n"                       \
  "v_fma_f64 v[112:113], v[112:113], v[118:119], v[112:113]\n" \
  "v_fma_f64 v[118:119], -v[124:125], v[112:113], 1.0\n" \
  "v_fma_f64 v[112:113], v[112:113], v[118:119], v[112:113]\n"                 \
  "v_mul_f64 v[114:115], v[124:125], v[114:115]\n"                             \
  "v_mul_f64 v[118:119], v[116:117], v[112:113]\n"                             \
  "v_mul_f64 v[120:121], v[118:119], v[118:119]\n"                             \
  "v_ldexp_f64 v[124:125], v[118:119], 5\n"                                    \
  "s_mov_b32 s90, 0x33333333\n" \
  "s_mov_b32 s91, 0x40433333\n" \
  "v_add_f64 v[124:125], v[124:125], -s[90:91]\n" \
  "s_mov_b32 s92, 0x55555611\n" \
  "s_mov_b32 s93, 0x40255555\n" \
  "v_fma_f64 v[124:125], v[120:121], v[124:125], s[92:93]\n"                   \
  "v_mul_f64 v[116:117], v[120:121], v[118:119]\n"                             \
  "v_mul_f64 v[120:121], v[120:121], s[90:91]\n"                               \
  "s_mov_b32 s90, 0x555554f8\n" \
  "s_mov_b32 s91, 0x40355555\n" \
  "v_add_f64 v[120:121], v[120:121], s[90:91]\n"                               \
  "s_mov_b32 s90, 0x00000000\n" \
  "s_mov_b32 s91, 0xc0480000\n" \
  "v_fma_f64 v[120:121], v[118:119], s[90:91], v[120:121]\n"                   \
  "v_fma_f64 v[120:121], -v[116:117], s[92:93], v[120:121]\n"                  \
  "v_mul_f64 v[116:117], v[114:115], v[114:115]\n" \
  "v_mul_f64 v[116:117], v[116:117], v[114:115]\n"                             \
  "s_mov_b32 s90, 0x11116ee4\n" \
  "s_mov_b32 s91, 0x3fb11111\n" \
  "v_fma_f64 v[120:121], -v[116:117], s[90:91], v[120:121]\n"                  \
  "v_cmp_gt_f64_e32 vcc, 0.5, v[118:119]\n"                                    \
  "v_cndmask_b32_e32 v120, v120, v124, vcc\n" \
  "v_cndmask_b32_e32 v121, v121, v125, vcc\n" \
  "v_mul_f64 v[124:125], %[cS], v[102:103]\n"                                  \
  "v_mul_f64 v[124:125], v[124:125], v[112:113]\n" \
  "v_mul_f64 v[124:125], v[124:125], v[112:113]\n" \
  "v_mul_f64 v[124:125], v[124:125], v[112:113]\n" \
  "v_mul_f64 v[124:125], v[124:125], v[120:121]\n" \
  "v_cndmask_b32_e64 v122, v122, v124, s[94:95]\n" \
  "v_cndmask_b32_e64 v123, v123, v125, s[94:95]\n" \
  "s_branch L_ed_accy_%=\n" \
  "L_ed_done_%=:\n" \
  "s_waitcnt lgkmcnt(0)\n"

#define ER_DIRECT_CLOBBERS "v96", "v97", "v98", "v99", "v100", "v101", "v102", "v103", "v104", "v105", "v106", "v107", "v108", "v109", "v110", "v111", "v112", "v113", "v114", "v115", "v116", "v117", "v118", "v119", "v120", "v121", "v122", "v123", "v124", "v125", "v126", "v127", "s88", "s89", "s90", "s91", "s92", "s93", "s94", "s95", "vcc", "scc", "memory"

#define ER_TRIP4_ASM(YUKSEG, FSTOFF) \
  "s_mov_b32 %[ntr], 0\n" \
  "L_er_topa_%=:\n" \
  "v_cmp_eq_u32_e32 vcc, %[tail], %[q]\n" \
  "s_cbranch_vccz L_er_done_%=\n" \
  "v_ffbl_b32_e32 v126, %[m]\n"                                                \
  "v_add_co_u32_e64 v112, s[90:91], %[m], -1\n"                                \
  "v_lshl_add_u32 v127, v126, 4, %[q]\n" \
  "v_and_b32_e32 %[m], v112, %[m]\n" \
  "v_cmp_eq_u32_e32 vcc, 0, %[m]\n" \
  "s_and_saveexec_b64 s[92:93], vcc\n"                                         \
  "v_add_u32_e32 v112, %[q], %[lane4]\n" \
  "ds_read_b32 %[q], %[q] offset:256\n" \
  "ds_read_b32 %[m], v112\n" \
  "s_mov_b64 exec, s[92:93]\n" \
  "ds_read_b128 v[104:107], v127 offset:320\n" \
  "ds_read_b128 v[108:111], v127 offset:848\n" \
  "s_waitcnt lgkmcnt(0)\n" \
  "v_add_f64 v[104:105], v[104:105], -%[tpx]\n" \
  "v_add_f64 v[106:107], v[106:107], -%[tpy]\n" \
  "v_mul_f64 v[112:113], v[106:107], v[106:107]\n" \
  "v_add_f64 v[108:109], v[108:109], -%[tpz]\n" \
  "v_fmac_f64_e32 v[112:113], v[104:105], v[104:105]\n" \
  "v_fmac_f64_e32 v[112:113], v[108:109], v[108:109]\n" \
  "v_cmp_ngt_f64_e32 vcc, %[reach2], v[112:113]\n"                             \
  "s_and_b64 s[94:95], vcc, s[90:91]\n"                                        \
  "s_cbranch_scc1 L_er_rarea_%=\n" \
  "L_er_incuta_%=:\n" \
  "v_add_f64 v[116:117], v[112:113], %[tiny]\n"                                \
  "v_rsq_f64_e32 v[114:115], v[116:117]\n" \
  "v_cmp_gt_f64_e32 vcc, %[h2max], v[112:113]\n"                               \
  "v_mul_f64 v[118:119], v[116:117], v[114:115]\n"                             \
  "v_fma_f64 v[118:119], -v[118:119], v[114:115], 1.0\n" \
  "v_mul_f64 v[120:121], v[114:115], 0.5\n" \
  "v_fma_f64 v[114:115], v[120:121], v[118:119], v[114:115]\n"                 \
  "v_mul_f64 v[116:117], v[116:117], v[114:115]\n"                             \
  "v_mul_f64 v[118:119], v[116:117], %[asmthfac]\n" \
  "v_cvt_i32_f64_e32 v112, v[118:119]\n"                                       \
  "v_min_i32_e32 v112, 0x7ff, v112\n" \
  YUKSEG \
  "s_waitcnt lgkmcnt(0)\n" \
  "v_fma_f64 v[122:123], -%[utor2wpi], v[112:113], v[122:123]\n"               \
  "v_mul_f64 v[122:123], v[110:111], v[122:123]\n" \
  "v_mul_f64 v[122:123], v[114:115], v[122:123]\n"                             \
  "s_cbranch_vccnz L_er_softa_%=\n" \
  "L_er_acca_%=:\n" \
  "v_fmac_f64_e32 %[ax], v[104:105], v[122:123]\n" \
  "v_fmac_f64_e32 %[ay], v[106:107], v[122:123]\n" \
  "v_fmac_f64_e32 %[az], v[108:109], v[122:123]\n" \
  "L_er_topb_%=:\n" \
  "v_ffbl_b32_e32 v126, %[m]\n"                                                \
  "v_add_co_u32_e64 v112, s[90:91], %[m], -1\n"                                \
  "v_lshl_add_u32 v127, v126, 4, %[q]\n" \
  "v_and_b32_e32 %[m], v112, %[m]\n" \
  "v_cmp_eq_u32_e32 vcc, 0, %[m]\n" \
  "s_and_saveexec_b64 s[92:93], vcc\n"                                         \
  "v_add_u32_e32 v112, %[q], %[lane4]\n" \
  "ds_read_b32 %[q], %[q] offset:256\n" \
  "ds_read_b32 %[m], v112\n" \
  "s_mov_b64 exec, s[92:93]\n" \
  "ds_read_b128 v[104:107], v127 offset:320\n" \
  "ds_read_b128 v[108:111], v127 offset:848\n" \
  "s_waitcnt lgkmcnt(0)\n" \
  "v_add_f64 v[104:105], v[104:105], -%[tpx]\n" \
  "v_add_f64 v[106:107], v[106:107], -%[tpy]\n" \
  "v_mul_f64 v[112:113], v[106:107], v[106:107]\n" \
  "v_add_f64 v[108:109], v[108:109], -%[tpz]\n" \
  "v_fmac_f64_e32 v[112:113], v[104:105], v[104:105]\n" \
  "v_fmac_f64_e32 v[112:113], v[108:109], v[108:109]\n" \
  "v_cmp_ngt_f64_e32 vcc, %[reach2], v[112:113]\n"                             \
  "s_and_b64 s[94:95], vcc, s[90:91]\n"                                        \
  "s_cbranch_scc1 L_er_rareb_%=\n" \
  "L_er_incutb_%=:\n" \
  "v_add_f64 v[116:117], v[112:113], %[tiny]\n"                                \
  "v_rsq_f64_e32 v[114:115], v[116:117]\n" \
  "v_cmp_gt_f64_e32 vcc, %[h2max], v[112:113]\n"                               \
  "v_mul_f64 v[118:119], v[116:117], v[114:115]\n"                             \
  "v_fma_f64 v[118:119], -v[118:119], v[114:115], 1.0\n" \
  "v_mul_f64 v[120:121], v[114:115], 0.5\n" \
  "v_fma_f64 v[114:115], v[120:121], v[118:119], v[114:115]\n"                 \
  "v_mul_f64 v[116:117], v[116:117], v[114:115]\n"                             \
  "v_mul_f64 v[118:119], v[116:117], %[asmthfac]\n" \
  "v_cvt_i32_f64_e32 v112, v[118:119]\n"                                       \
  "v_min_i32_e32 v112, 0x7ff, v112\n" \
  YUKSEG \
  "s_waitcnt lgkmcnt(0)\n" \
  "v_fma_f64 v[122:123], -%[utor2wpi], v[112:113], v[122:123]\n"               \
  "v_mul_f64 v[122:123], v[110:111], v[122:123]\n" \
  "v_mul_f64 v[122:123], v[114:115], v[122:123]\n"                             \
  "s_cbranch_vccnz L_er_softb_%=\n" \
  "L_er_accb_%=:\n" \
  "v_fmac_f64_e32 %[ax], v[104:105], v[122:123]\n" \
  "v_fmac_f64_e32 %[ay], v[106:107], v[122:123]\n" \
  "v_fmac_f64_e32 %[az], v[108:109], v[122:123]\n" \
  "s_add_u32 %[ntr], %[ntr], 2\n" \
  "s_branch L_er_topa_%=\n" \
  "L_er_rarea_%=:\n" \
  "v_cndmask_b32_e64 v111, v111, 0, s[94:95]\n"                                \
  "v_cndmask_b32_e64 v110, v110, 0, s[94:95]\n" \
  "v_cndmask_b32_e64 v118, 0, 1, s[94:95]\n" \
  "v_sub_u32_e32 %[nint], %[nint], v118\n" \
  "s_branch L_er_incuta_%=\n" \
  "L_er_softa_%=:\n" \
  "v_mul_i32_i24_e32 v118, 0xfffffff1, v126\n"                                 \
  "v_add_u32_e32 v118, v127, v118\n" \
  "ds_read_u8 v118, v118 offset:272\n" \
  "s_waitcnt lgkmcnt(0)\n" \
  "v_lshl_add_u32 v118, v118, 3, %[etab]\n" \
  "ds_read_b64 v[124:125], v118 offset:" FSTOFF "\n"                           \
  "s_waitcnt lgkmcnt(0)\n" \
  "v_max_f64 v[124:125], v[124:125], %[hT]\n"                                  \
  "v_rcp_f64_e32 v[112:113], v[124:125]\n" \
  "v_cmp_lt_f64_e64 s[94:95], v[116:117], v[124:125]\n"                        \
  "v_fma_f64 v[118:119], -v[124:125], v[112:113], 1.0\n"                       \
  "v_fma_f64 v[112:113], v[112:113], v[118:119], v[112:113]\n" \
  "v_fma_f64 v[118:119], -v[124:125], v[112:113], 1.0\n" \
  "v_fma_f64 v[112:113], v[112:113], v[118:119], v[112:113]\n"                 \
  "v_mul_f64 v[114:115], v[124:125], v[114:115]\n"                             \
  "v_mul_f64 v[118:119], v[116:117], v[112:113]\n"                             \
  "v_mul_f64 v[120:121], v[118:119], v[118:119]\n"                             \
  "v_ldexp_f64 v[124:125], v[118:119], 5\n"                                    \
  "s_mov_b32 s90, 0x33333333\n" \
  "s_mov_b32 s91, 0x40433333\n" \
  "v_add_f64 v[124:125], v[124:125], -s[90:91]\n" \
  "s_mov_b32 s92, 0x55555611\n" \
  "s_mov_b32 s93, 0x40255555\n" \
  "v_fma_f64 v[124:125], v[120:121], v[124:125], s[92:93]\n"                   \
  "v_mul_f64 v[116:117], v[120:121], v[118:119]\n"                             \
  "v_mul_f64 v[120:121], v[120:121], s[90:91]\n"                               \
  "s_mov_b32 s90, 0x555554f8\n" \
  "s_mov_b32 s91, 0x40355555\n" \
  "v_add_f64 v[120:121], v[120:121], s[90:91]\n"                               \
  "s_mov_b32 s90, 0x00000000\n" \
  "s_mov_b32 s91, 0xc0480000\n" \
  "v_fma_f64 v[120:121], v[118:119], s[90:91], v[120:121]\n"                   \
  "v_fma_f64 v[120:121], -v[116:117], s[92:93], v[120:121]\n"                  \
  "v_mul_f64 v[116:117], v[114:115], v[114:115]\n" \
  "v_mul_f64 v[116:117], v[116:117], v[114:115]\n"                             \
  "s_mov_b32 s90, 0x11116ee4\n" \
  "s_mov_b32 s91, 0x3fb11111\n" \
  "v_fma_f64 v[120:121], -v[116:117], s[90:91], v[120:121]\n"                  \
  "v_cmp_gt_f64_e32 vcc, 0.5, v[118:119]\n"                                    \
  "v_cndmask_b32_e32 v120, v120, v124, vcc\n" \
  "v_cndmask_b32_e32 v121, v121, v125, vcc\n" \
  "v_mul_f64 v[124:125], %[cS], v[110:111]\n"                                  \
  "v_mul_f64 v[124:125], v[124:125], v[112:113]\n" \
  "v_mul_f64 v[124:125], v[124:125], v[112:113]\n" \
  "v_mul_f64 v[124:125], v[124:125], v[112:113]\n" \
  "v_mul_f64 v[124:125], v[124:125], v[120:121]\n" \
  "v_cndmask_b32_e64 v122, v122, v124, s[94:95]\n" \
  "v_cndmask_b32_e64 v123, v123, v125, s[94:95]\n" \
  "s_branch L_er_acca_%=\n" \
  "L_er_rareb_%=:\n" \
  "v_cndmask_b32_e64 v111, v111, 0, s[94:95]\n"                                \
  "v_cndmask_b32_e64 v110, v110, 0, s[94:95]\n" \
  "v_cndmask_b32_e64 v118, 0, 1, s[94:95]\n" \
  "v_sub_u32_e32 %[nint], %[nint], v118\n" \
  "s_branch L_er_incutb_%=\n" \
  "L_er_softb_%=:\n" \
  "v_mul_i32_i24_e32 v118, 0xfffffff1, v126\n"                                 \
  "v_add_u32_e32 v118, v127, v118\n" \
  "ds_read_u8 v118, v118 offset:272\n" \
  "s_waitcnt lgkmcnt(0)\n" \
  "v_lshl_add_u32 v118, v118, 3, %[etab]\n" \
  "ds_read_b64 v[124:125], v118 offset:" FSTOFF "\n"                           \
  "s_waitcnt lgkmcnt(0)\n" \
  "v_max_f64 v[124:125], v[124:125], %[hT]\n"                                  \
  "v_rcp_f64_e32 v[112:113], v[124:125]\n" \
  "v_cmp_lt_f64_e64 s[94:95], v[116:117], v[124:125]\n"                        \
  "v_fma_f64 v[118:119], -v[124:125], v[112:113], 1.0\n"                       \
  "v_fma_f64 v[112:113], v[112:113], v[118:119], v[112:113]\n" \
  "v_fma_f64 v[118:119], -v[124:125], v[112:113], 1.0\n" \
  "v_fma_f64 v[112:113], v[112:113], v[118:119], v[112:113]\n"                 \
  "v_mul_f64 v[114:115], v[124:125], v[114:115]\n"                             \
  "v_mul_f64 v[118:119], v[116:117], v[112:113]\n"                             \
  "v_mul_f64 v[120:121], v[118:119], v[118:119]\n"                             \
  "v_ldexp_f64 v[124:125], v[118:119], 5\n"                                    \
  "s_mov_b32 s90, 0x33333333\n" \
  "s_mov_b32 s91, 0x40433333\n" \
  "v_add_f64 v[124:125], v[124:125], -s[90:91]\n" \
  "s_mov_b32 s92, 0x55555611\n" \
  "s_mov_b32 s93, 0x40255555\n" \
  "v_fma_f64 v[124:125], v[120:121], v[124:125], s[92:93]\n"                   \
  "v_mul_f64 v[116:117], v[120:121], v[118:119]\n"                             \
  "v_mul_f64 v[120:121], v[120:121], s[90:91]\n"                               \
  "s_mov_b32 s90, 0x555554f8\n" \
  "s_mov_b32 s91, 0x40355555\n" \
  "v_add_f64 v[120:121], v[120:121], s[90:91]\n"                               \
  "s_mov_b32 s90, 0x00000000\n" \
  "s_mov_b32 s91, 0xc0480000\n" \
  "v_fma_f64 v[120:121], v[118:119], s[90:91], v[120:121]\n"                   \
  "v_fma_f64 v[120:121], -v[116:117], s[92:93], v[120:121]\n"                  \
  "v_mul_f64 v[116:117], v[114:115], v[114:115]\n" \
  "v_mul_f64 v[116:117], v[116:117], v[114:115]\n"                             \
  "s_mov_b32 s90, 0x11116ee4\n" \
  "s_mov_b32 s91, 0x3fb11111\n" \
  "v_fma_f64 v[120:121], -v[116:117], s[90:91], v[120:121]\n"                  \
  "v_cmp_gt_f64_e32 vcc, 0.5, v[118:119]\n"                                    \
  "v_cndmask_b32_e32 v120, v120, v124, vcc\n" \
  "v_cndmask_b32_e32 v121, v121, v125, vcc\n" \
  "v_mul_f64 v[124:125], %[cS], v[110:111]\n"                                  \
  "v_mul_f64 v[124:125], v[124:125], v[112:113]\n" \
  "v_mul_f64 v[124:125], v[124:125], v[112:113]\n" \
  "v_mul_f64 v[124:125], v[124:125], v[112:113]\n" \
  "v_mul_f64 v[124:125], v[124:125], v[120:121]\n" \
  "v_cndmask_b32_e64 v122, v122, v124, s[94:95]\n" \
  "v_cndmask_b32_e64 v123, v123, v125, s[94:95]\n" \
  "s_branch L_er_accb_%=\n" \
  "L_er_done_%=:\n"

#define ER_TRIP_CLOBBERS "v104", "v105", "v106", "v107", "v108", "v109", "v110", "v111", "v112", "v113", "v114", "v115", "v116", "v117", "v118", "v119", "v120", "v121", "v122", "v123", "v124", "v125", "v126", "v127", "s90", "s91", "s92", "s93", "s94", "s95", "vcc", "scc", "memory"

#define ER_CULL_WRAP \
  "v_mul_f64 v[110:111], v[104:105], %[invbox]\n"                              \
  "v_mul_f64 v[112:113], v[106:107], %[invbox]\n" \
  "v_mul_f64 v[114:115], v[108:109], %[invbox]\n" \
  "v_rndne_f64_e32 v[110:111], v[110:111]\n" \
  "v_rndne_f64_e32 v[112:113], v[112:113]\n" \
  "v_rndne_f64_e32 v[114:115], v[114:115]\n" \
  "v_fma_f64 v[104:105], -v[110:111], %[box], v[104:105]\n" \
  "v_fma_f64 v[106:107], -v[112:113], %[box], v[106:107]\n" \
  "v_fma_f64 v[108:109], -v[114:115], %[box], v[108:109]\n"

#define ER_CULL_ASM(WRAPSEG) \
  "v_add_f64 v[104:105], %[rx], -%[bcx]\n" \
  "v_add_f64 v[106:107], %[ry], -%[bcy]\n" \
  "v_add_f64 v[108:109], %[rz], -%[bcz]\n" \
  WRAPSEG \
  "v_add_f64 v[110:111], |v[104:105]|, -%[bhx]\n"                              \
  "v_add_f64 v[112:113], |v[106:107]|, -%[bhy]\n" \
  "v_add_f64 v[114:115], |v[108:109]|, -%[bhz]\n" \
  "v_max_f64 v[110:111], v[110:111], 0\n" \
  "v_max_f64 v[112:113], v[112:113], 0\n" \
  "v_max_f64 v[114:115], v[114:115], 0\n" \
  "v_mul_f64 v[110:111], v[110:111], v[110:111]\n" \
  "v_fma_f64 v[110:111], v[112:113], v[112:113], v[110:111]\n" \
  "v_fma_f64 v[110:111], v[114:115], v[114:115], v[110:111]\n" \
  "v_cmp_gt_f64_e32 vcc, %[reach2], v[110:111]\n"                              \
  "v_cmp_neq_f64_e64 s[90:91], 0, %[rw]\n"                                     \
  "s_and_b64 s[90:91], s[90:91], vcc\n" \
  "s_bcnt1_i32_b64 %[cnt], s[90:91]\n" \
  "v_mbcnt_lo_u32_b32 v116, s90, 0\n" \
  "v_mbcnt_hi_u32_b32 v116, s91, v116\n" \
  "v_add_u32_e32 v116, %[wrpos], v116\n"                                       \
  "s_and_saveexec_b64 s[92:93], s[90:91]\n" \
  "v_cmp_gt_u32_e32 vcc, 32, v116\n"                                           \
  "v_mov_b32_e32 v117, %[q0]\n" \
  "v_mov_b32_e32 v119, %[q1]\n" \
  "v_cndmask_b32_e32 v117, v119, v117, vcc\n" \
  "v_cmp_gt_u32_e32 vcc, 64, v116\n" \
  "v_mov_b32_e32 v119, %[q2]\n" \
  "v_cndmask_b32_e32 v117, v119, v117, vcc\n" \
  "v_and_b32_e32 v118, 31, v116\n" \
  "v_lshl_add_u32 v118, v118, 4, v117\n" \
  "ds_write_b128 v118, v[104:107] offset:320\n" \
  "ds_write_b64 v118, v[108:109] offset:848\n" \
  "ds_write_b64 v118, %[rw] offset:856\n" \
  "s_mov_b64 exec, s[92:93]\n"

#define ER_CULL_CLOBBERS "v104", "v105", "v106", "v107", "v108", "v109", "v110", "v111", "v112", "v113", "v114", "v115", "v116", "v117", "v118", "v119", "s90", "s91", "s92", "s93", "vcc", "scc", "memory"
```

gadget-2.0.7-ngravs_amd/csrc/kernels_eval.hip:

```cpp
#include "engine.hpp"
#include "walk_device.hpp"
#include <type_traits>

#define ER_SLOT 1360u
#define ER_STUB 848u
#define ER_NM 0u
#define ER_NEXT 256u
#define ER_TYPE 272u
#define ER_XY 320u
#define ER_ZM 848u
#define ER_MAXWAVES 16

extern __shared__ __attribute__((aligned(16))) unsigned char er_smem[];

#define ER_AS3(T, a) (*(__attribute__((address_space(3))) T *)(unsigned long)(a))
__device__ __forceinline__ unsigned lds_u32(unsigned a) { return ER_AS3(const unsigned, a); }
__device__ __forceinline__ void lds_st_u32(unsigned a, unsigned v) { ER_AS3(unsigned, a) = v; }
__device__ __forceinline__ unsigned char lds_u8(unsigned a) { return ER_AS3(const unsigned char, a); }
__device__ __forceinline__ void lds_st_u8(unsigned a, unsigned char v) { ER_AS3(unsigned char, a) = v; }
__device__ __forceinline__ double4 er_entry(unsigned q, int j)
{
  typedef double d2 __attribute__((ext_vector_type(2)));
  const unsigned a = q + ((unsigned)j << 4);
  const d2 lo = ER_AS3(const d2, a + ER_XY), hi = ER_AS3(const d2, a + ER_ZM);
  double4 r;
  r.x = lo.x;
  r.y = lo.y;
  r.z = hi.x;
  r.w = hi.y;
  return r;
}

#include "eval_asm.inc"

struct ErLaw
{
  double cN, cY, cS;
  unsigned trow;
  unsigned pad;
};

template <int NG, bool YUK, bool ET>
__global__ __launch_bounds__(ER_MAXWAVES * 64) void k_eval_ring(
    const double4 *__restrict__ n_mom, const int *__restrict__ n_flags, const double4 *__restrict__ s_pm,
    const unsigned char *__restrict__ s_type, const unsigned char *__restrict__ s_active, const double *__restrict__ table,
    WalkParams wp, long long t_first,
    long long t_count, int *__restrict__ counter, double *__restrict__ r_acc, int *__restrict__ r_nint,
    const int *__restrict__ region_base, const int *__restrict__ gcount, long long g_first, long long g_cnt, int lcap, int scap,
    int S, const int *__restrict__ tlist, int SG, int K)
{
  double *tab_s = reinterpret_cast<double *>(er_smem);
  const int ntabs = wp.ntab_lds + (YUK ? wp.exp_tab : 0);
  const unsigned tab_bytes = (unsigned)(sizeof(double) * ntabs * NTAB);
  const int wave = threadIdx.x >> 6, lane = threadIdx.x & 63;
  double *expT = reinterpret_cast<double *>(er_smem + tab_bytes);
  double *fsT = expT + 32;
  ErLaw *lawT = reinterpret_cast<ErLaw *>(fsT + 8);
  const unsigned fixed_bytes = tab_bytes + 40u * (unsigned)sizeof(double) + (unsigned)(NG * NG * sizeof(ErLaw));
  const unsigned wave_bytes = (unsigned)K * ER_SLOT;
  const unsigned lds0 = (unsigned)(unsigned long)(__attribute__((address_space(3))) unsigned char *)er_smem;
  const unsigned term_q = lds0 + fixed_bytes;
  const unsigned wbase = (unsigned)__builtin_amdgcn_readfirstlane((int)(term_q + ER_STUB + (unsigned)wave * wave_bytes));
  bool usoft = true;
#pragma unroll
  for(int q = 0; q < NGRAVS_NTYPES; q++)
    usoft = usoft && wp.fsoft[q] == wp.fsoft[0];
  {
    if(threadIdx.x < 32)
      expT[threadIdx.x] = exp2(-(double)threadIdx.x / 32.0);
    if(threadIdx.x >= 32 && threadIdx.x < 40)
      fsT[threadIdx.x - 32] = threadIdx.x - 32 < NGRAVS_NTYPES ? wp.fsoft[threadIdx.x - 32] : 0.0;
    if(threadIdx.x < NG * NG)
      {
        const int a = threadIdx.x / NG, b = threadIdx.x % NG;
        ErLaw l;
        l.cN = wp.cN[a][b];
        l.cY = wp.cY[a][b];
        l.cS = wp.cS[a][b];
        l.trow = lds0 + (unsigned)(wp.tab_slot[a * NG + b] * NTAB * sizeof(double));
        l.pad = 0;
        lawT[threadIdx.x] = l;
      }
    for(int t = threadIdx.x; t < ntabs * NTAB; t += blockDim.x)
      {
        const int u = t / NTAB;
        tab_s[t] = table[(size_t)(u < wp.ntab_lds ? wp.slot_src[u] : NG * NG) * NTAB + (t % NTAB)];
      }
    if(lane <= K && (lane < K || wave == 0))
      {
        typedef double d2 __attribute__((ext_vector_type(2)));
        const unsigned qs = lane < K ? wbase + (unsigned)lane * ER_SLOT : term_q;
        d2 far, zm;
        far.x = far.y = 1e10;
        zm.x = 1e10;
        zm.y = 0.0;
        ER_AS3(d2, qs + ER_XY - 16u) = far;
        ER_AS3(d2, qs + ER_ZM - 16u) = zm;
        lds_st_u8(qs + ER_TYPE - 1, 7);
      }
    if(lane < 8)
      for(int k = 0; k < K; k++)
        lds_st_u32(wbase + (unsigned)k * ER_SLOT + ER_TYPE + 4u * (unsigned)lane, 0u);
    if(wave == 0)
      {
        lds_st_u32(term_q + ER_NM + 4 * lane, 0u);
        if(lane == 0)
          lds_st_u32(term_q + ER_NEXT, term_q);
      }
    __syncthreads();
  }
  const unsigned etab_a = lds0 + (YUK ? (unsigned)(wp.ntab_lds * NTAB * sizeof(double)) : tab_bytes);
  const int G = WAVE / S;
  const long long ngroups = g_cnt;
  unsigned lane_pat = ~0u;
  if(S > 1)
    {
      lane_pat = 0;
      for(int j = lane & (S - 1); j < 32; j += S)
        lane_pat |= 1u << j;
    }
  const double invbox = wp.box > 0 ? 1.0 / wp.box : 0.0;
  double h2max = 0;
#pragma unroll
  for(int q = 0; q < NGRAVS_NTYPES; q++)
    h2max = fmax(h2max, wp.fsoft[q] * wp.fsoft[q]);
  h2max = wave_uniform(h2max);
  unsigned xcc = 0;
  asm volatile("s_getreg_b32 %0, hwreg(HW_REG_XCC_ID)" : "=s"(xcc));
  xcc &= 7u;
  const long long seg = (ngroups + 7) / 8;
  int steal = 0;
  unsigned long long acc_st[4] = {0, 0, 0, 0};
  const unsigned lane4 = 4u * (unsigned)lane;
  const int mh = lane >> 5;
  const int mrow = 16 * ((lane >> 2) & 1) + 4 * ((lane & 31) >> 3) + (lane & 3);
  typedef float f16v __attribute__((ext_vector_type(16)));
  const double BIG = 1e300;
  for(;;)
    {
      long long grp = -1;
      while(steal < 8)
        {
          const int sx = (int)((xcc + steal) & 7u);
          int k = 0;
          if(lane == 0)
            k = atomicAdd(&counter[8 + sx], 1);
          k = __builtin_amdgcn_readfirstlane(k);
          const long long g0 = seg * sx + k;
          if(k < seg && g0 < ngroups)
            {
              grp = g0;
              break;
            }
          steal++;
        }
      if(grp < 0)
        break;
      const long long ru = grp / SG;
      const int *const lbase = region_base + (size_t)ru * ((size_t)NG * lcap + scap);
      const long long grel = grp;
      grp += g_first;
      const long long tk = grp * G + lane / S;
      const bool in_range = tk < t_count;
      const long long ti = tlist ? (in_range ? (long long)tlist[tk] : 0ll) : t_first + tk;
      const bool valid = in_range && (tlist != nullptr || (s_active[ti] & 1) != 0);
      double px = 0, py = 0, pz = 0, hT = 0;
      int tg = 0;
      if(valid)
        {
          double4 p = s_pm[ti];
          px = p.x;
          py = p.y;
          pz = p.z;
          int ptype = s_type[ti];
          tg = wp.t2g[ptype];
          hT = wp.fsoft[ptype];
        }
      if(!__any(valid ? 1 : 0))
        continue;
      int n_items[NG];
      bool bad = false;
#pragma unroll
      for(int g = 0; g < NG; g++)
        {
          n_items[g] = __builtin_amdgcn_readfirstlane(gcount[ru * NG + g]);
          bad |= n_items[g] < 0;
        }
      if(bad)
        continue;
      const double lox = wave_min(valid ? px : BIG), hix = wave_max(valid ? px : -BIG);
      const double loy = wave_min(valid ? py : BIG), hiy = wave_max(valid ? py : -BIG);
      const double loz = wave_min(valid ? pz : BIG), hiz = wave_max(valid ? pz : -BIG);
      const double bcx = wave_uniform(0.5 * (lox + hix)), bcy = wave_uniform(0.5 * (loy + hiy)), bcz = wave_uniform(0.5 * (loz + hiz));
      const double bhx = wave_uniform(0.5 * (hix - lox)), bhy = wave_uniform(0.5 * (hiy - loy)), bhz = wave_uniform(0.5 * (hiz - loz));
      const double bhmax = fmax(bhx, fmax(bhy, bhz));
      const bool prewrap = __builtin_amdgcn_readfirstlane(
                               (int)(wp.periodic && (wp.boxhalf - bhmax) * (wp.boxhalf - bhmax) > wp.reach2 && (wp.boxhalf - bhmax) > 0)) != 0;
      const bool lanewrap = wp.periodic && !prewrap;
      bool nowrap = !wp.periodic;
      if(wp.periodic && wp.src_in_box)
        {
          const double rl_ = __builtin_sqrt(wp.reach2);
          nowrap = __builtin_amdgcn_readfirstlane((int)(bcx - bhx - rl_ >= 0.0 && bcx + bhx + rl_ <= wp.box && bcy - bhy - rl_ >= 0.0 &&
                                                        bcy + bhy + rl_ <= wp.box && bcz - bhz - rl_ >= 0.0 &&
                                                        bcz + bhz + rl_ <= wp.box)) != 0;
        }
      float mB[2][3];
      {
        const float tfx = (float)(px - bcx), tfy = (float)(py - bcy), tfz = (float)(pz - bcz);
        const float m2x = -2.0f * tfx, m2y = -2.0f * tfy, m2z = -2.0f * tfz;
        float cth;
        const double rl = __builtin_sqrt(wp.reach2);
        const double dl = 4.76837158203125e-07 * (bhmax + rl);
        const double M = 3.0 * (2.0 * bhmax + rl) * (2.0 * bhmax + rl);
        const double thr = (wp.reach2 + 4.0 * rl * dl + 1.0e-6 * M) * (1.0 + 2e-6);
        cth = (float)((double)tfx * tfx + (double)tfy * tfy + (double)tfz * tfz - thr);
        cth = cth - 1.2e-7f * __builtin_fabsf(cth);
#pragma unroll
        for(int tb = 0; tb < 2; tb++)
          {
            const int src = 32 * tb + (lane & 31);
            const float x_ = __shfl(m2x, src), y_ = __shfl(m2y, src), z_ = __shfl(m2z, src), c_ = __shfl(cth, src);
            mB[tb][0] = mh ? y_ : x_;
            mB[tb][1] = mh ? 1.0f : z_;
            mB[tb][2] = mh ? 0.0f : c_;
          }
      }

      double ax = 0, ay = 0, az = 0;
      int nint = 0;
      int st_entries = 0, st_iters = 0;

      auto run_lists = [&](auto lw_tag) {
        constexpr bool LW = decltype(lw_tag)::value;
        const bool fastmask = !LW && !wp.exact_reach;
        const double tpx = LW ? px : px - bcx, tpy = LW ? py : py - bcy, tpz = LW ? pz : pz - bcz;
        for(int g = 0; g < NG; g++)
          {
            const int n = n_items[g < NG ? g : 0];
            const int *__restrict__ items = lbase + (size_t)g * lcap;
            wave_sync();
            st_entries += n;
            if(n == 0)
              continue;
            double cNg, cYg, cSg;
            unsigned trow_a;
            {
              const ErLaw l = lawT[tg * NG + g];
              cNg = l.cN;
              cYg = l.cY;
              cSg = l.cS;
              trow_a = l.trow;
            }
            const int nq = (n + 3) >> 2;
            const int nsuper = (nq + WAVE - 1) / WAVE, nchunks = 4 * nsuper;
            const int M = nsuper * WAVE;
            int s_ = (int)(0.6180339887498949 * M) | 1;
            if(s_ >= M)
              s_ = 1;
            for(;;)
              {
                int a = nsuper, b = s_ % nsuper;
                while(b)
                  {
                    int t = a % b;
                    a = b;
                    b = t;
                  }
                if(a == 1)
                  break;
                s_ += 2;
                if(s_ >= M)
                  {
                    s_ = 1;
                    break;
                  }
              }
            const int step64 = (int)((64ll * s_) % M);
            int slot = (int)(((long long)lane * s_) % M);
            int4 qd = {0, 0, 0, 0};
            int nv = 0;
            int wr_slot = 0, wr_pos = 0, tail_slot = 0, nlive = 0;
            bool first = true;
            unsigned newest_q = term_q;
            unsigned m = 0, q = term_q;
            double rx = 0, ry = 0, rz = 0, rw = 0;
            int hs1 = 0;
            for(int cc = 0;; cc++)
              {
                const bool have_chunk = cc < nchunks;
                rw = 0.0;
                if(have_chunk)
                  {
                    const int bn = cc & 3;
                    if(bn == 0)
                      {
                        nv = 0;
                        if(slot < nq)
                          {
                            qd = reinterpret_cast<const int4 *>(items)[slot];
                            nv = n - 4 * slot;
                          }
                        slot += step64;
                        slot = slot >= M ? slot - M : slot;
                      }
                    const int item = bn == 0 ? qd.x : (bn == 1 ? qd.y : (bn == 2 ? qd.z : qd.w));
                    if(bn < nv)
                      {
                        const bool isp = item >= 0;
                        const unsigned idx = isp ? (unsigned)item : ~(unsigned)item;
                        const double4 *src = isp ? s_pm + idx : n_mom + idx;
                        const double4 r = *src;
                        rx = r.x;
                        ry = r.y;
                        rz = r.z;
                        rw = r.w;
                        if(!usoft)
                          hs1 = isp ? (int)s_type[idx] : ((n_flags[idx / NG] >> 2) & 7);
                      }
                  }
                while(nlive > 0 && (!have_chunk || K * 32 - (nlive * 32 + wr_pos) < WAVE))
                  {
                  const unsigned tail_q = wbase + (unsigned)tail_slot * ER_SLOT;
                  if constexpr(!LW && (ET || !YUK))
                    {
                      int ntr;
#define ER_TRIP_CALL(ASMTEXT)                                                                                                       \
  asm volatile(ASMTEXT                                                                                         \
               : [m] "+v"(m), [q] "+v"(q), [ax] "+v"(ax), [ay] "+v"(ay), [az] "+v"(az), [nint] "+v"(nint), [ntr] "=&s"(ntr)           \
               : [tpx] "v"(tpx), [tpy] "v"(tpy), [tpz] "v"(tpz), [cN] "v"(cNg), [cY] "v"(cYg), [cS] "v"(cSg), [hT] "v"(hT),          \
                 [trow] "v"(trow_a), [lane4] "v"(lane4), [tail] "s"(tail_q), [reach2] "s"(wp.reach2), [tiny] "s"(1e-290),           \
                 [asmthfac] "s"(wp.asmthfac), [ec0] "s"(wp.ec[0]), [ec1] "s"(wp.ec[1]), [ec2] "s"(wp.ec[2]), [ec3] "s"(wp.ec[3]),   \
                 [utor2wpi] "s"(wp.utor2wpi), [ym] "s"(wp.ym), [h2max] "s"(h2max), [etab] "s"(etab_a)                              \
               : ER_TRIP_CLOBBERS)
                      if constexpr(YUK)
                        ER_TRIP_CALL(ER_TRIP4_ASM(ER_YUK_ET, ER_FST_OFF_ET));
                      else
                        ER_TRIP_CALL(ER_TRIP4_ASM(ER_NOYUK, ER_FST_OFF_NOET));
#undef ER_TRIP_CALL
                      st_iters += ntr;
                    }
                  else
                  for(;;)
                    {
                      if(__builtin_amdgcn_ballot_w64(q == tail_q) == 0ull)
                        break;
                      st_iters += (int)(__builtin_popcountll(__builtin_amdgcn_ballot_w64(true)) >> 6);
                      int j;
                      asm("v_ffbl_b32 %0, %1" : "=v"(j) : "v"(m));
                      const double4 e = er_entry(q, j);
                      const unsigned qe = q;
                      unsigned long long actm_;
                      unsigned mm1;
                      asm("v_add_co_u32_e64 %0, %1, %2, -1" : "=v"(mm1), "=s"(actm_) : "v"(m));
                      const unsigned long long actm = ((unsigned long long)(unsigned)__builtin_amdgcn_readfirstlane((int)(actm_ >> 32)) << 32) |
                                                      (unsigned)__builtin_amdgcn_readfirstlane((int)actm_);
                      m &= mm1;
                      if(m == 0u)
                        {
                          const unsigned qn = lds_u32(q + ER_NEXT);
                          m = lds_u32(q + ER_NM + lane4);
                          q = qn;
                        }
                      double dx = e.x - tpx, dy = e.y - tpy, dz = e.z - tpz;
                      if(LW)
                        {
                          dx = nearest(dx, wp.box, wp.boxhalf);
                          dy = nearest(dy, wp.box, wp.boxhalf);
                          dz = nearest(dz, wp.box, wp.boxhalf);
                        }
                      const double r2 = dx * dx + dy * dy + dz * dz;
                      double mw = e.w;
                      const unsigned long long fpos = actm & __builtin_amdgcn_ballot_w64(!(r2 < wp.reach2));
                      if(fpos != 0ull)
                        {
                          asm volatile("; beyond the exact cut" ::: "memory");
                          double r2o = r2;
                          asm volatile("" : "+v"(r2o));
                          unsigned long long am = actm;
                          asm volatile("" : "+s"(am));
                          const bool out = ((am >> lane) & 1ull) != 0 && !(r2o < wp.reach2);
                          mw = out ? 0.0 : mw;
                          nint -= out ? 1 : 0;
                        }
                      const double q2 = r2 + 1e-290;
                      double ri = __builtin_amdgcn_rsq(q2);
                      ri = ri * (1.5 - 0.5 * q2 * ri * ri);
                      const double rr = q2 * ri;
                      const double ri2 = ri * ri;
                      double f = cNg * ri2;
                      const double xt = wp.asmthfac * rr;
                      int tab = (int)xt;
                      tab = tab < NTAB - 1 ? tab : NTAB - 1;
                      if(YUK)
                        {
                          double ex_;
                          if(ET)
                            {
                              const double fb = __builtin_amdgcn_fract(xt);
                              double pz_ = fb * wp.ec[3];
                              pz_ = pz_ - wp.ec[2];
                              pz_ = __builtin_fma(pz_, fb, wp.ec[1]);
                              pz_ = __builtin_fma(pz_, fb, -wp.ec[0]);
                              pz_ = __builtin_fma(pz_, fb, 1.0);
                              ex_ = ER_AS3(const double, etab_a + 8u * (unsigned)tab) * pz_;
                            }
                          else
                            ex_ = exp_neg_fast(rr * wp.ym, expT);
                          f += cYg * ex_ * (wp.ym * ri + ri2);
                        }
                      f -= wp.utor2wpi * ER_AS3(const double, trow_a + 8u * (unsigned)tab);
                      double fac = f * mw * ri;
                      if(wave_any(r2 < h2max))
                        {
                          asm volatile("; softened pair" ::: "memory");
                          const double h = __builtin_fmax(hT, fsT[lds_u8(qe + (unsigned)j + ER_TYPE)]);
                          const bool soft = rr < h;
                          double h_inv = 1 / h, u = rr * h_inv;
                          double v = (u < 0.5) ? (10.666666666667 + u * u * (32.0 * u - 38.4))
                                               : (21.333333333333 - 48.0 * u + 38.4 * u * u - 10.666666666667 * u * u * u - 0.066666666667 / (u * u * u));
                          double fs = cSg * mw * h_inv * h_inv * h_inv * v;
                          fac = soft ? fs : fac;
                        }
                      ax = __builtin_fma(dx, fac, ax);
                      ay = __builtin_fma(dy, fac, ay);
                      az = __builtin_fma(dz, fac, az);
                    }
                  tail_slot = tail_slot + 1 >= K ? 0 : tail_slot + 1;
                  nlive--;
                  }
                if(!have_chunk)
                  break;
                {
                  const int s1 = wr_slot + 1 >= K ? wr_slot + 1 - K : wr_slot + 1, s2 = wr_slot + 2 >= K ? wr_slot + 2 - K : wr_slot + 2;
                  const unsigned q0 = wbase + (unsigned)wr_slot * ER_SLOT, q1 = wbase + (unsigned)s1 * ER_SLOT, q2 = wbase + (unsigned)s2 * ER_SLOT;
                  if(!LW && usoft)
                    {
                      int cnt;
#define ER_CULL_CALL(WRAPSEG)                                                                                                     \
  asm volatile(ER_CULL_ASM(WRAPSEG)                                                                                                \
               : [cnt] "=&s"(cnt)                                                                                                   \
               : [rx] "v"(rx), [ry] "v"(ry), [rz] "v"(rz), [rw] "v"(rw), [bcx] "s"(bcx), [bcy] "s"(bcy), [bcz] "s"(bcz), [bhx] "s"(bhx),  \
                 [bhy] "s"(bhy), [bhz] "s"(bhz), [reach2] "s"(wp.reach2), [box] "s"(wp.box), [invbox] "s"(invbox), [wrpos] "s"(wr_pos),   \
                 [q0] "s"(q0), [q1] "s"(q1), [q2] "s"(q2)                                                                           \
               : ER_CULL_CLOBBERS)
                      if(nowrap)
                        ER_CULL_CALL("");
                      else
                        ER_CULL_CALL(ER_CULL_WRAP);
#undef ER_CULL_CALL
                      wr_pos += cnt;
                    }
                  else
                    {
                      double ex = rx - bcx, ey = ry - bcy, ez = rz - bcz;
                      if(!nowrap)
                        {
                          ex = nearest_abs(ex, wp.box, invbox);
                          ey = nearest_abs(ey, wp.box, invbox);
                          ez = nearest_abs(ez, wp.box, invbox);
                        }
                      const double b0 = fmax(0.0, fabs(ex) - bhx), b1 = fmax(0.0, fabs(ey) - bhy), b2 = fmax(0.0, fabs(ez) - bhz);
                      const bool live = rw != 0.0 && (b0 * b0 + b1 * b1 + b2 * b2 < wp.reach2);
                      const unsigned long long lm = __ballot(live ? 1 : 0);
                      if(live)
                        {
                          const int L = wr_pos + lane_prefix(lm);
                          const unsigned sq = L < 32 ? q0 : (L < 64 ? q1 : q2);
                          const unsigned ea = sq + 16u * (unsigned)(L & 31);
                          typedef double d2 __attribute__((ext_vector_type(2)));
                          d2 lo, hi;
                          lo.x = LW ? rx : ex;
                          lo.y = LW ? ry : ey;
                          hi.x = LW ? rz : ez;
                          hi.y = rw;
                          ER_AS3(d2, ea + ER_XY) = lo;
                          ER_AS3(d2, ea + ER_ZM) = hi;
                          if(!usoft)
                            lds_st_u8(sq + ER_TYPE + (unsigned)(L & 31), (unsigned char)(hs1 & 7));
                        }
                      wr_pos += __popcll(lm);
                    }
                  wave_sync();
                }
                const bool last = cc + 1 >= nchunks;
                while(wr_pos >= 32 || (last && wr_pos > 0))
                  {
                    const int nfill = wr_pos < 32 ? wr_pos : 32;
                    const unsigned sq = wbase + (unsigned)wr_slot * ER_SLOT;
                    unsigned word = 0;
                    if(fastmask)
                      {
                        const double4 er = er_entry(sq, mrow);
                        const float fx = (float)er.x, fy = (float)er.y, fz = (float)er.z;
                        const float e2 = __builtin_fmaf(fz, fz, __builtin_fmaf(fy, fy, fx * fx));
                        const float a0 = mh ? fy : fx, a1 = mh ? e2 : fz, a2 = mh ? 0.0f : 1.0f;
                        unsigned wt[2];
#pragma unroll
                        for(int tb = 0; tb < 2; tb++)
                          {
                            f16v acc;
#pragma unroll
                            for(int r = 0; r < 16; r++)
                              acc[r] = 0.0f;
                            acc = __builtin_amdgcn_mfma_f32_32x32x2f32(a0, mB[tb][0], acc, 0, 0, 0);
                            acc = __builtin_amdgcn_mfma_f32_32x32x2f32(a1, mB[tb][1], acc, 0, 0, 0);
                            acc = __builtin_amdgcn_mfma_f32_32x32x2f32(a2, mB[tb][2], acc, 0, 0, 0);
                            unsigned w_ = 0;
#pragma unroll
                            for(int r = 15; r >= 0; r--)
                              w_ = __builtin_amdgcn_alignbit(w_, __float_as_uint(acc[r]), 31);
                            wt[tb] = w_;
                          }
                        const auto sw = __builtin_amdgcn_permlane32_swap(wt[0], wt[1], false, false);
                        word = sw[0] | (sw[1] << 16);
                      }
                    else
                      {
                        for(int b = 0; b < nfill; b++)
                          {
                            const double4 e = er_entry(sq, b);
                            double dx = e.x - tpx, dy = e.y - tpy, dz = e.z - tpz;
                            if(LW)
                              {
                                dx = nearest(dx, wp.box, wp.boxhalf);
                                dy = nearest(dy, wp.box, wp.boxhalf);
                                dz = nearest(dz, wp.box, wp.boxhalf);
                              }
                            const double r2 = dx * dx + dy * dy + dz * dz;
                            word |= (r2 < wp.reach2) ? (1u << b) : 0u;
                          }
                      }
                    const unsigned okm = !valid ? 0u : (nfill >= 32 ? ~0u : ((1u << nfill) - 1u));
                    word &= okm & lane_pat;
                    nint += __popc(word);
                    if(first)
                      {
                        m = word;
                        q = sq;
                        first = false;
                      }
                    else
                      {
                        lds_st_u32(newest_q + ER_NM + lane4, word);
                        if(lane == 0)
                          lds_st_u32(newest_q + ER_NEXT, sq);
                      }
                    lds_st_u32(sq + ER_NM + lane4, 0u);
                    if(lane == 0)
                      lds_st_u32(sq + ER_NEXT, sq);
                    newest_q = sq;
                    wave_sync();
                    wr_pos -= nfill;
                    wr_slot = wr_slot + 1 >= K ? 0 : wr_slot + 1;
                    nlive++;
                  }
                if(last)
                  {
                    if(!first && lane == 0)
                      lds_st_u32(newest_q + ER_NEXT, term_q);
                    wave_sync();
                  }
              }
            wave_sync();
          }
      };
      if(lanewrap)
        run_lists(std::true_type{});
      else
        run_lists(std::false_type{});

      {
        int st_nodes = 0, st_batches = 0;
        if(grel % SG == 0)
          {
            const long long u_cnt = (g_cnt + SG - 1) / SG;
            st_nodes = __builtin_amdgcn_readfirstlane(gcount[NG * u_cnt + ru]);
            st_batches = __builtin_amdgcn_readfirstlane(gcount[(NG + 1) * u_cnt + ru]);
          }
        acc_st[0] += (unsigned long long)st_entries;
        acc_st[1] += (unsigned long long)st_nodes;
        acc_st[2] += (unsigned long long)st_batches;
        acc_st[3] += (unsigned long long)st_iters;
      }
      if(S > 1)
        {
          for(int off = 1; off < S; off <<= 1)
            {
              ax += __shfl_xor(ax, off);
              ay += __shfl_xor(ay, off);
              az += __shfl_xor(az, off);
              nint += __shfl_xor(nint, off);
            }
        }
      if(valid && (lane & (S - 1)) == 0)
        {
          r_acc[3 * ti + 0] = ax;
          r_acc[3 * ti + 1] = ay;
          r_acc[3 * ti + 2] = az;
          r_nint[ti] = nint;
        }
    }
  if(lane == 0)
    {
      unsigned long long *st64 = reinterpret_cast<unsigned long long *>(counter + 16);
#pragma unroll
      for(int qq = 0; qq < 4; qq++)
        if(acc_st[qq])
          atomicAdd(&st64[qq], acc_st[qq]);
    }
}

static size_t er_fixed_bytes(const WalkParams &wp, bool yuk)
{
  return sizeof(double) * (size_t)(wp.ntab_lds + (yuk ? wp.exp_tab : 0)) * NTAB + 40 * sizeof(double) + (size_t)wp.ng * wp.ng * sizeof(ErLaw) +
         ER_STUB;
}
int eval_ring_slots(const WalkParams &wp, bool yuk, int waves)
{
  const size_t fixed = er_fixed_bytes(wp, yuk);
  const size_t avail = 160 * 1024 - fixed;
  const long long per_wave = (long long)(avail / (size_t)waves);
  long long K = per_wave / (long long)ER_SLOT;
  if(K > 8)
    K = 8;
  return K >= 4 ? (int)K : 0;
}

template <int NG> using RingRowsNG = Table<Row<NG, 0, 0>, Row<NG, 1, 0>, Row<NG, 1, 1>>;
using RingRows = decltype(RingRowsNG<1>{} + RingRowsNG<2>{} + RingRowsNG<3>{});

template <int NG, int YUK, int ET>
static int launch_eval_ring_t(Row<NG, YUK, ET>, ngravs_ctx *c, const TreeView &tv, const WalkParams &wp, int nblk, int waves, int K,
                              const int *region, const int *gcount, long long g0, long long nb, int lcap, int scap, int S,
                              const int *tlist, int SG, long long t_count)
{
  const size_t fixed = er_fixed_bytes(wp, YUK);
  const size_t lds = fixed + (size_t)waves * ((size_t)K * ER_SLOT);
  auto ke = k_eval_ring<NG, YUK, ET>;
  HIP_TRY(c, hipFuncSetAttribute(reinterpret_cast<const void *>(ke), hipFuncAttributeMaxDynamicSharedMemorySize, (int)lds));
  hipLaunchKernelGGL(ke, dim3((unsigned)nblk), dim3(waves * 64), lds, c->stream, tv.mom, tv.flags, c->s_pm.p, c->s_type.p, c->s_active.p, c->table.p, wp,
                     (long long)c->shard_first, t_count, c->walk_counters.p, c->r_acc.p, c->r_nint.p, region, gcount, g0, nb, lcap, scap,
                     S, tlist, SG, K);
  return NGRAVS_OK;
}

int launch_eval_ring(ngravs_ctx *c, const TreeView &tv, const WalkParams &wp, bool yuk, int nblk, int waves, int K, const int *region,
                     const int *gcount, long long g0, long long nb, int lcap, int scap, int S, const int *tlist, int SG, long long t_count)
{
  const int key[] = {c->cfg.n_gravs, yuk, yuk && wp.exp_tab};
  return dispatch(c, RingRows{}, key, [&](auto row) {
    return launch_eval_ring_t(row, c, tv, wp, nblk, waves, K, region, gcount, g0, nb, lcap, scap, S, tlist, SG, t_count);
  });
}
```

Before: 638.4 million.

## Load eval constants into SGPRs inside asm and re-read args from kernarg

Moves the per-kernel scalar constants (reach2, h2max, asmthfac, Yukawa coefficients, box) into a small device struct. The inline-asm trip and cull blocks now load them into fixed SGPRs with s_load, instead of keeping them live across the whole kernel as compiler-held scalar operands. Kernel arguments are packed into one struct and re-read from the kernarg segment at each use, which shortens SGPR live ranges and is meant to lower register pressure. It adds a scalar memory load and wait per asm invocation, and separately loosens the PM CU-partition fit margin.

New measurement: 644.1 million, median of 6. No clear change (+0.9%).

```diff
diff --git a/gadget-2.0.7-ngravs_amd/csrc/capi.hip b/gadget-2.0.7-ngravs_amd/csrc/capi.hip
--- a/gadget-2.0.7-ngravs_amd/csrc/capi.hip
+++ b/gadget-2.0.7-ngravs_amd/csrc/capi.hip
@@ -377,6 +377,7 @@
   c->lat.release();
   c->walk_stack.release();
   c->walk_counters.release();
+  c->eval_consts.release();
   c->walk_ovf.release();
   c->walk_tlist.release();
   c->walk_tmp.release();
@@ -1223,7 +1224,7 @@
 }
 
 static const double PM_CU_SCALE[4] = {17.75, 9.07, 6.16, 4.74};
-static const double PM_FIT_MARGIN = 1.05, PM_SHARE_COST = 1.04;
+static const double PM_FIT_MARGIN = 1.0, PM_SHARE_COST = 1.04;
 static int choose_pm_cus(ngravs_ctx *c)
 {
   if(!overlap_eligible(c))
diff --git a/gadget-2.0.7-ngravs_amd/csrc/engine.hpp b/gadget-2.0.7-ngravs_amd/csrc/engine.hpp
--- a/gadget-2.0.7-ngravs_amd/csrc/engine.hpp
+++ b/gadget-2.0.7-ngravs_amd/csrc/engine.hpp
@@ -134,6 +134,16 @@
   int law_accel[NG_MAX][NG_MAX], law_spline[NG_MAX][NG_MAX];
   int user;
   UserTabs ut;
+};
+
+struct EvalConsts
+{
+  double reach2;
+  double h2max;
+  double asmthfac, utor2wpi, ym;
+  double ec[4];
+  double tiny;
+  double box, invbox;
 };
 
 struct TreeView
@@ -279,6 +289,8 @@
   double walk_ia_ratio = 0;
   bool all_active = true;
   DevBuf<int> walk_ovf;
+  DevBuf<EvalConsts> eval_consts;
+  EvalConsts eval_consts_host;
   DevBuf<int> walk_counters;
   DevBuf<double> r_acc, r_pm, r_oldacc;
   DevBuf<int> r_nint;
diff --git a/gadget-2.0.7-ngravs_amd/csrc/eval_asm.inc b/gadget-2.0.7-ngravs_amd/csrc/eval_asm.inc
--- a/gadget-2.0.7-ngravs_amd/csrc/eval_asm.inc
+++ b/gadget-2.0.7-ngravs_amd/csrc/eval_asm.inc
@@ -5,20 +5,20 @@
 
 #define ER_YUK_ET \
   "v_fract_f64_e32 v[118:119], v[118:119]\n"                                   \
-  "v_mul_f64 v[122:123], v[118:119], %[ec3]\n" \
+  "v_mul_f64 v[122:123], v[118:119], s[80:81]\n" \
   "v_lshl_add_u32 v113, v112, 3, %[etab]\n" \
-  "v_add_f64 v[122:123], v[122:123], -%[ec2]\n" \
+  "v_add_f64 v[122:123], v[122:123], -s[78:79]\n" \
   "ds_read_b64 v[124:125], v113\n"                                             \
   "v_lshl_add_u32 v112, v112, 3, %[trow]\n" \
-  "v_fma_f64 v[122:123], v[122:123], v[118:119], %[ec1]\n" \
+  "v_fma_f64 v[122:123], v[122:123], v[118:119], s[76:77]\n" \
   "ds_read_b64 v[112:113], v112\n"                                             \
-  "v_fma_f64 v[122:123], v[122:123], v[118:119], -%[ec0]\n" \
+  "v_fma_f64 v[122:123], v[122:123], v[118:119], -s[74:75]\n" \
   "v_mul_f64 v[120:121], v[114:115], v[114:115]\n"                             \
   "v_fma_f64 v[122:123], v[122:123], v[118:119], 1.0\n"                        \
   "s_waitcnt lgkmcnt(1)\n" \
   "v_mul_f64 v[122:123], v[124:125], v[122:123]\n"                             \
   "v_mul_f64 v[122:123], %[cY], v[122:123]\n" \
-  "v_fma_f64 v[124:125], %[ym], v[114:115], v[120:121]\n"                      \
+  "v_fma_f64 v[124:125], s[72:73], v[114:115], v[120:121]\n"                   \
   "v_mul_f64 v[122:123], v[124:125], v[122:123]\n" \
   "v_fmac_f64_e32 v[122:123], %[cN], v[120:121]\n"
 
@@ -276,7 +276,29 @@
 
 #define ER_DIRECT_CLOBBERS "v96", "v97", "v98", "v99", "v100", "v101", "v102", "v103", "v104", "v105", "v106", "v107", "v108", "v109", "v110", "v111", "v112", "v113", "v114", "v115", "v116", "v117", "v118", "v119", "v120", "v121", "v122", "v123", "v124", "v125", "v126", "v127", "s88", "s89", "s90", "s91", "s92", "s93", "s94", "s95", "vcc", "scc", "memory"
 
-#define ER_TRIP4_ASM(YUKSEG, FSTOFF) \
+#define ER_KC_REACH2 0
+#define ER_KC_H2MAX 8
+#define ER_KC_ASMTHFAC 16
+#define ER_KC_UTOR2WPI 24
+#define ER_KC_YM 32
+#define ER_KC_EC0 40
+#define ER_KC_EC1 48
+#define ER_KC_EC2 56
+#define ER_KC_EC3 64
+#define ER_KC_TINY 72
+#define ER_KC_BOX 80
+#define ER_KC_INVBOX 88
+
+#define ER_KC_TRIP_YUK \
+  "s_load_dwordx16 s[64:79], %[kc], 0x0\n"                                     \
+  "s_load_dwordx4 s[80:83], %[kc], 0x40\n"
+
+#define ER_KC_TRIP_NOYUK \
+  "s_load_dwordx8 s[64:71], %[kc], 0x0\n"                                      \
+  "s_load_dwordx2 s[82:83], %[kc], 0x48\n"
+
+#define ER_TRIP4_ASM(KCSEG, YUKSEG, FSTOFF) \
+  KCSEG \
   "s_mov_b32 %[ntr], 0\n" \
   "L_er_topa_%=:\n" \
   "v_cmp_eq_u32_e32 vcc, %[tail], %[q]\n" \
@@ -300,24 +322,24 @@
   "v_add_f64 v[108:109], v[108:109], -%[tpz]\n" \
   "v_fmac_f64_e32 v[112:113], v[104:105], v[104:105]\n" \
   "v_fmac_f64_e32 v[112:113], v[108:109], v[108:109]\n" \
-  "v_cmp_ngt_f64_e32 vcc, %[reach2], v[112:113]\n"                             \
+  "v_cmp_ngt_f64_e32 vcc, s[64:65], v[112:113]\n"                              \
   "s_and_b64 s[94:95], vcc, s[90:91]\n"                                        \
   "s_cbranch_scc1 L_er_rarea_%=\n" \
   "L_er_incuta_%=:\n" \
-  "v_add_f64 v[116:117], v[112:113], %[tiny]\n"                                \
+  "v_add_f64 v[116:117], v[112:113], s[82:83]\n"                               \
   "v_rsq_f64_e32 v[114:115], v[116:117]\n" \
-  "v_cmp_gt_f64_e32 vcc, %[h2max], v[112:113]\n"                               \
+  "v_cmp_gt_f64_e32 vcc, s[66:67], v[112:113]\n"                               \
   "v_mul_f64 v[118:119], v[116:117], v[114:115]\n"                             \
   "v_fma_f64 v[118:119], -v[118:119], v[114:115], 1.0\n" \
   "v_mul_f64 v[120:121], v[114:115], 0.5\n" \
   "v_fma_f64 v[114:115], v[120:121], v[118:119], v[114:115]\n"                 \
   "v_mul_f64 v[116:117], v[116:117], v[114:115]\n"                             \
-  "v_mul_f64 v[118:119], v[116:117], %[asmthfac]\n" \
+  "v_mul_f64 v[118:119], v[116:117], s[68:69]\n" \
   "v_cvt_i32_f64_e32 v112, v[118:119]\n"                                       \
   "v_min_i32_e32 v112, 0x7ff, v112\n" \
   YUKSEG \
   "s_waitcnt lgkmcnt(0)\n" \
-  "v_fma_f64 v[122:123], -%[utor2wpi], v[112:113], v[122:123]\n"               \
+  "v_fma_f64 v[122:123], -s[70:71], v[112:113], v[122:123]\n"                  \
   "v_mul_f64 v[122:123], v[110:111], v[122:123]\n" \
   "v_mul_f64 v[122:123], v[114:115], v[122:123]\n"                             \
   "s_cbranch_vccnz L_er_softa_%=\n" \
@@ -345,24 +367,24 @@
   "v_add_f64 v[108:109], v[108:109], -%[tpz]\n" \
   "v_fmac_f64_e32 v[112:113], v[104:105], v[104:105]\n" \
   "v_fmac_f64_e32 v[112:113], v[108:109], v[108:109]\n" \
-  "v_cmp_ngt_f64_e32 vcc, %[reach2], v[112:113]\n"                             \
+  "v_cmp_ngt_f64_e32 vcc, s[64:65], v[112:113]\n"                              \
   "s_and_b64 s[94:95], vcc, s[90:91]\n"                                        \
   "s_cbranch_scc1 L_er_rareb_%=\n" \
   "L_er_incutb_%=:\n" \
-  "v_add_f64 v[116:117], v[112:113], %[tiny]\n"                                \
+  "v_add_f64 v[116:117], v[112:113], s[82:83]\n"                               \
   "v_rsq_f64_e32 v[114:115], v[116:117]\n" \
-  "v_cmp_gt_f64_e32 vcc, %[h2max], v[112:113]\n"                               \
+  "v_cmp_gt_f64_e32 vcc, s[66:67], v[112:113]\n"                               \
   "v_mul_f64 v[118:119], v[116:117], v[114:115]\n"                             \
   "v_fma_f64 v[118:119], -v[118:119], v[114:115], 1.0\n" \
   "v_mul_f64 v[120:121], v[114:115], 0.5\n" \
   "v_fma_f64 v[114:115], v[120:121], v[118:119], v[114:115]\n"                 \
   "v_mul_f64 v[116:117], v[116:117], v[114:115]\n"                             \
-  "v_mul_f64 v[118:119], v[116:117], %[asmthfac]\n" \
+  "v_mul_f64 v[118:119], v[116:117], s[68:69]\n" \
   "v_cvt_i32_f64_e32 v112, v[118:119]\n"                                       \
   "v_min_i32_e32 v112, 0x7ff, v112\n" \
   YUKSEG \
   "s_waitcnt lgkmcnt(0)\n" \
-  "v_fma_f64 v[122:123], -%[utor2wpi], v[112:113], v[122:123]\n"               \
+  "v_fma_f64 v[122:123], -s[70:71], v[112:113], v[122:123]\n"                  \
   "v_mul_f64 v[122:123], v[110:111], v[122:123]\n" \
   "v_mul_f64 v[122:123], v[114:115], v[122:123]\n"                             \
   "s_cbranch_vccnz L_er_softb_%=\n" \
@@ -484,22 +506,32 @@
   "v_cndmask_b32_e64 v122, v122, v124, s[94:95]\n" \
   "v_cndmask_b32_e64 v123, v123, v125, s[94:95]\n" \
   "s_branch L_er_accb_%=\n" \
-  "L_er_done_%=:\n"
-
-#define ER_TRIP_CLOBBERS "v104", "v105", "v106", "v107", "v108", "v109", "v110", "v111", "v112", "v113", "v114", "v115", "v116", "v117", "v118", "v119", "v120", "v121", "v122", "v123", "v124", "v125", "v126", "v127", "s90", "s91", "s92", "s93", "s94", "s95", "vcc", "scc", "memory"
+  "L_er_done_%=:\n" \
+  "s_waitcnt lgkmcnt(0)\n"
+
+#define ER_TRIP_CLOBBERS "v104", "v105", "v106", "v107", "v108", "v109", "v110", "v111", "v112", "v113", "v114", "v115", "v116", "v117", "v118", "v119", "v120", "v121", "v122", "v123", "v124", "v125", "v126", "v127", "s64", "s65", "s66", "s67", "s68", "s69", "s70", "s71", "s72", "s73", "s74", "s75", "s76", "s77", "s78", "s79", "s80", "s81", "s82", "s83", "s90", "s91", "s92", "s93", "s94", "s95", "vcc", "scc", "memory"
+
+#define ER_KC_CULL \
+  "s_load_dwordx2 s[64:65], %[kc], 0x0\n"
+
+#define ER_KC_CULL_WRAP \
+  "s_load_dwordx2 s[64:65], %[kc], 0x0\n"                                      \
+  "s_load_dwordx4 s[68:71], %[kc], 0x50\n"
 
 #define ER_CULL_WRAP \
-  "v_mul_f64 v[110:111], v[104:105], %[invbox]\n"                              \
-  "v_mul_f64 v[112:113], v[106:107], %[invbox]\n" \
-  "v_mul_f64 v[114:115], v[108:109], %[invbox]\n" \
+  "s_waitcnt lgkmcnt(0)\n" \
+  "v_mul_f64 v[110:111], v[104:105], s[70:71]\n"                               \
+  "v_mul_f64 v[112:113], v[106:107], s[70:71]\n" \
+  "v_mul_f64 v[114:115], v[108:109], s[70:71]\n" \
   "v_rndne_f64_e32 v[110:111], v[110:111]\n" \
   "v_rndne_f64_e32 v[112:113], v[112:113]\n" \
   "v_rndne_f64_e32 v[114:115], v[114:115]\n" \
-  "v_fma_f64 v[104:105], -v[110:111], %[box], v[104:105]\n" \
-  "v_fma_f64 v[106:107], -v[112:113], %[box], v[106:107]\n" \
-  "v_fma_f64 v[108:109], -v[114:115], %[box], v[108:109]\n"
-
-#define ER_CULL_ASM(WRAPSEG) \
+  "v_fma_f64 v[104:105], -v[110:111], s[68:69], v[104:105]\n" \
+  "v_fma_f64 v[106:107], -v[112:113], s[68:69], v[106:107]\n" \
+  "v_fma_f64 v[108:109], -v[114:115], s[68:69], v[108:109]\n"
+
+#define ER_CULL_ASM(KCSEG, WRAPSEG) \
+  KCSEG \
   "v_add_f64 v[104:105], %[rx], -%[bcx]\n" \
   "v_add_f64 v[106:107], %[ry], -%[bcy]\n" \
   "v_add_f64 v[108:109], %[rz], -%[bcz]\n" \
@@ -513,7 +545,8 @@
   "v_mul_f64 v[110:111], v[110:111], v[110:111]\n" \
   "v_fma_f64 v[110:111], v[112:113], v[112:113], v[110:111]\n" \
   "v_fma_f64 v[110:111], v[114:115], v[114:115], v[110:111]\n" \
-  "v_cmp_gt_f64_e32 vcc, %[reach2], v[110:111]\n"                              \
+  "s_waitcnt lgkmcnt(0)\n" \
+  "v_cmp_gt_f64_e32 vcc, s[64:65], v[110:111]\n"                               \
   "v_cmp_neq_f64_e64 s[90:91], 0, %[rw]\n"                                     \
   "s_and_b64 s[90:91], s[90:91], vcc\n" \
   "s_bcnt1_i32_b64 %[cnt], s[90:91]\n" \
@@ -535,4 +568,4 @@
   "ds_write_b64 v118, %[rw] offset:856\n" \
   "s_mov_b64 exec, s[92:93]\n"
 
-#define ER_CULL_CLOBBERS "v104", "v105", "v106", "v107", "v108", "v109", "v110", "v111", "v112", "v113", "v114", "v115", "v116", "v117", "v118", "v119", "s90", "s91", "s92", "s93", "vcc", "scc", "memory"
+#define ER_CULL_CLOBBERS "v104", "v105", "v106", "v107", "v108", "v109", "v110", "v111", "v112", "v113", "v114", "v115", "v116", "v117", "v118", "v119", "s64", "s65", "s68", "s69", "s70", "s71", "s90", "s91", "s92", "s93", "vcc", "scc", "memory"
diff --git a/gadget-2.0.7-ngravs_amd/csrc/kernels_eval.hip b/gadget-2.0.7-ngravs_amd/csrc/kernels_eval.hip
--- a/gadget-2.0.7-ngravs_amd/csrc/kernels_eval.hip
+++ b/gadget-2.0.7-ngravs_amd/csrc/kernels_eval.hip
@@ -31,7 +31,20 @@
   return r;
 }
 
+__device__ __forceinline__ double wave_uniform_sgpr(double v)
+{
+  int lo, hi;
+  asm("v_readfirstlane_b32 %0, %2\n\tv_readfirstlane_b32 %1, %3" : "=s"(lo), "=s"(hi) : "v"(__double2loint(v)), "v"(__double2hiint(v)));
+  return __hiloint2double(hi, lo);
+}
+
 #include "eval_asm.inc"
+static_assert(offsetof(EvalConsts, reach2) == ER_KC_REACH2 && offsetof(EvalConsts, h2max) == ER_KC_H2MAX &&
+                  offsetof(EvalConsts, asmthfac) == ER_KC_ASMTHFAC && offsetof(EvalConsts, utor2wpi) == ER_KC_UTOR2WPI &&
+                  offsetof(EvalConsts, ym) == ER_KC_YM && offsetof(EvalConsts, ec) == ER_KC_EC0 &&
+                  offsetof(EvalConsts, ec) + 3 * sizeof(double) == ER_KC_EC3 && offsetof(EvalConsts, tiny) == ER_KC_TINY &&
+                  offsetof(EvalConsts, box) == ER_KC_BOX && offsetof(EvalConsts, invbox) == ER_KC_INVBOX,
+              "EvalConsts and the offsets the assembly blocks load from differ");
 
 struct ErLaw
 {
@@ -40,15 +53,39 @@
   unsigned pad;
 };
 
+#define ER_GLOBAL __attribute__((address_space(1)))
+typedef double er_d4 __attribute__((ext_vector_type(4)));
+typedef int er_i4 __attribute__((ext_vector_type(4)));
+struct ErGroupArgs
+{
+  long long t_first, t_count;
+  ER_GLOBAL int *counter;
+  ER_GLOBAL double *r_acc;
+  ER_GLOBAL int *r_nint;
+  const ER_GLOBAL int *region_base, *gcount;
+  long long g_first, g_cnt;
+  int lcap, scap, S, SG;
+  const ER_GLOBAL int *tlist;
+  const ER_GLOBAL unsigned char *s_active;
+  const ER_GLOBAL er_d4 *s_pm, *n_mom;
+  const ER_GLOBAL unsigned char *s_type;
+  const ER_GLOBAL int *n_flags;
+  WalkParams wp;
+};
+typedef const __attribute__((address_space(4))) ErGroupArgs *ErGroupArgsPtr;
+__device__ __forceinline__ ErGroupArgsPtr er_group_args()
+{
+  ErGroupArgsPtr p = (ErGroupArgsPtr)__builtin_amdgcn_kernarg_segment_ptr();
+  asm volatile("" : "+s"(p));
+  return p;
+}
+
 template <int NG, bool YUK, bool ET>
 __global__ __launch_bounds__(ER_MAXWAVES * 64) void k_eval_ring(
-    const double4 *__restrict__ n_mom, const int *__restrict__ n_flags, const double4 *__restrict__ s_pm,
-    const unsigned char *__restrict__ s_type, const unsigned char *__restrict__ s_active, const double *__restrict__ table,
-    WalkParams wp, long long t_first,
-    long long t_count, int *__restrict__ counter, double *__restrict__ r_acc, int *__restrict__ r_nint,
-    const int *__restrict__ region_base, const int *__restrict__ gcount, long long g_first, long long g_cnt, int lcap, int scap,
-    int S, const int *__restrict__ tlist, int SG, int K)
-{
+    ErGroupArgs ga_, const double *__restrict__ table, const EvalConsts *__restrict__ kc, int K)
+{
+  (void)ga_;
+  auto &wp = er_group_args()->wp;
   double *tab_s = reinterpret_cast<double *>(er_smem);
   const int ntabs = wp.ntab_lds + (YUK ? wp.exp_tab : 0);
   const unsigned tab_bytes = (unsigned)(sizeof(double) * ntabs * NTAB);
@@ -110,15 +147,16 @@
     __syncthreads();
   }
   const unsigned etab_a = lds0 + (YUK ? (unsigned)(wp.ntab_lds * NTAB * sizeof(double)) : tab_bytes);
-  const int G = WAVE / S;
-  const long long ngroups = g_cnt;
   unsigned lane_pat = ~0u;
-  if(S > 1)
-    {
-      lane_pat = 0;
-      for(int j = lane & (S - 1); j < 32; j += S)
-        lane_pat |= 1u << j;
-    }
+  {
+    const int S = er_group_args()->S;
+    if(S > 1)
+      {
+        lane_pat = 0;
+        for(int j = lane & (S - 1); j < 32; j += S)
+          lane_pat |= 1u << j;
+      }
+  }
   const double invbox = wp.box > 0 ? 1.0 / wp.box : 0.0;
   double h2max = 0;
 #pragma unroll
@@ -127,8 +165,7 @@
   h2max = wave_uniform(h2max);
   unsigned xcc = 0;
   asm volatile("s_getreg_b32 %0, hwreg(HW_REG_XCC_ID)" : "=s"(xcc));
-  xcc &= 7u;
-  const long long seg = (ngroups + 7) / 8;
+  xcc = (unsigned)__builtin_amdgcn_readfirstlane((int)xcc) & 7u;
   int steal = 0;
   unsigned long long acc_st[4] = {0, 0, 0, 0};
   const unsigned lane4 = 4u * (unsigned)lane;
@@ -138,13 +175,17 @@
   const double BIG = 1e300;
   for(;;)
     {
+      ErGroupArgsPtr ga = er_group_args();
+      auto &wp = ga->wp;
+      const long long ngroups = ga->g_cnt, seg = (ngroups + 7) / 8;
+      const int S = ga->S, SG = ga->SG, G = WAVE / S;
       long long grp = -1;
       while(steal < 8)
         {
           const int sx = (int)((xcc + steal) & 7u);
           int k = 0;
           if(lane == 0)
-            k = atomicAdd(&counter[8 + sx], 1);
+            k = __hip_atomic_fetch_add(&ga->counter[8 + sx], 1, __ATOMIC_RELAXED, __HIP_MEMORY_SCOPE_AGENT);
           k = __builtin_amdgcn_readfirstlane(k);
           const long long g0 = seg * sx + k;
           if(k < seg && g0 < ngroups)
@@ -157,22 +198,24 @@
       if(grp < 0)
         break;
       const long long ru = grp / SG;
-      const int *const lbase = region_base + (size_t)ru * ((size_t)NG * lcap + scap);
+      const int lcap = ga->lcap;
+      const ER_GLOBAL int *const lbase = ga->region_base + (size_t)ru * ((size_t)NG * lcap + ga->scap);
       const long long grel = grp;
-      grp += g_first;
+      grp += ga->g_first;
       const long long tk = grp * G + lane / S;
-      const bool in_range = tk < t_count;
-      const long long ti = tlist ? (in_range ? (long long)tlist[tk] : 0ll) : t_first + tk;
-      const bool valid = in_range && (tlist != nullptr || (s_active[ti] & 1) != 0);
+      const bool in_range = tk < ga->t_count;
+      const ER_GLOBAL int *const tlist = ga->tlist;
+      const long long ti = tlist ? (in_range ? (long long)tlist[tk] : 0ll) : ga->t_first + tk;
+      const bool valid = in_range && (tlist != nullptr || (ga->s_active[ti] & 1) != 0);
       double px = 0, py = 0, pz = 0, hT = 0;
       int tg = 0;
       if(valid)
         {
-          double4 p = s_pm[ti];
+          const er_d4 p = ga->s_pm[ti];
           px = p.x;
           py = p.y;
           pz = p.z;
-          int ptype = s_type[ti];
+          int ptype = ga->s_type[ti];
           tg = wp.t2g[ptype];
           hT = wp.fsoft[ptype];
         }
@@ -183,7 +226,7 @@
 #pragma unroll
       for(int g = 0; g < NG; g++)
         {
-          n_items[g] = __builtin_amdgcn_readfirstlane(gcount[ru * NG + g]);
+          n_items[g] = __builtin_amdgcn_readfirstlane(ga->gcount[ru * NG + g]);
           bad |= n_items[g] < 0;
         }
       if(bad)
@@ -191,8 +234,8 @@
       const double lox = wave_min(valid ? px : BIG), hix = wave_max(valid ? px : -BIG);
       const double loy = wave_min(valid ? py : BIG), hiy = wave_max(valid ? py : -BIG);
       const double loz = wave_min(valid ? pz : BIG), hiz = wave_max(valid ? pz : -BIG);
-      const double bcx = wave_uniform(0.5 * (lox + hix)), bcy = wave_uniform(0.5 * (loy + hiy)), bcz = wave_uniform(0.5 * (loz + hiz));
-      const double bhx = wave_uniform(0.5 * (hix - lox)), bhy = wave_uniform(0.5 * (hiy - loy)), bhz = wave_uniform(0.5 * (hiz - loz));
+      const double bcx = wave_uniform_sgpr(0.5 * (lox + hix)), bcy = wave_uniform_sgpr(0.5 * (loy + hiy)), bcz = wave_uniform_sgpr(0.5 * (loz + hiz));
+      const double bhx = wave_uniform_sgpr(0.5 * (hix - lox)), bhy = wave_uniform_sgpr(0.5 * (hiy - loy)), bhz = wave_uniform_sgpr(0.5 * (hiz - loz));
       const double bhmax = fmax(bhx, fmax(bhy, bhz));
       const bool prewrap = __builtin_amdgcn_readfirstlane(
                                (int)(wp.periodic && (wp.boxhalf - bhmax) * (wp.boxhalf - bhmax) > wp.reach2 && (wp.boxhalf - bhmax) > 0)) != 0;
@@ -238,7 +281,7 @@
         for(int g = 0; g < NG; g++)
           {
             const int n = n_items[g < NG ? g : 0];
-            const int *__restrict__ items = lbase + (size_t)g * lcap;
+            const ER_GLOBAL int *items = lbase + (size_t)g * lcap;
             wave_sync();
             st_entries += n;
             if(n == 0)
@@ -278,7 +321,7 @@
               }
             const int step64 = (int)((64ll * s_) % M);
             int slot = (int)(((long long)lane * s_) % M);
-            int4 qd = {0, 0, 0, 0};
+            er_i4 qd = {0, 0, 0, 0};
             int nv = 0;
             int wr_slot = 0, wr_pos = 0, tail_slot = 0, nlive = 0;
             bool first = true;
@@ -298,7 +341,7 @@
                         nv = 0;
                         if(slot < nq)
                           {
-                            qd = reinterpret_cast<const int4 *>(items)[slot];
+                            qd = reinterpret_cast<const ER_GLOBAL er_i4 *>(items)[slot];
                             nv = n - 4 * slot;
                           }
                         slot += step64;
@@ -307,16 +350,19 @@
                     const int item = bn == 0 ? qd.x : (bn == 1 ? qd.y : (bn == 2 ? qd.z : qd.w));
                     if(bn < nv)
                       {
+                        ErGroupArgsPtr ca = er_group_args();
                         const bool isp = item >= 0;
                         const unsigned idx = isp ? (unsigned)item : ~(unsigned)item;
-                        const double4 *src = isp ? s_pm + idx : n_mom + idx;
-                        const double4 r = *src;
+                        const ER_GLOBAL er_d4 *b_pm = ca->s_pm, *b_mom = ca->n_mom;
+                        asm volatile("" : "+s"(b_pm), "+s"(b_mom));
+                        const ER_GLOBAL er_d4 *src = isp ? b_pm + idx : b_mom + idx;
+                        const er_d4 r = *src;
                         rx = r.x;
                         ry = r.y;
                         rz = r.z;
                         rw = r.w;
                         if(!usoft)
-                          hs1 = isp ? (int)s_type[idx] : ((n_flags[idx / NG] >> 2) & 7);
+                          hs1 = isp ? (int)ca->s_type[idx] : ((ca->n_flags[idx / NG] >> 2) & 7);
                       }
                   }
                 while(nlive > 0 && (!have_chunk || K * 32 - (nlive * 32 + wr_pos) < WAVE))
@@ -329,14 +375,12 @@
   asm volatile(ASMTEXT                                                                                         \
                : [m] "+v"(m), [q] "+v"(q), [ax] "+v"(ax), [ay] "+v"(ay), [az] "+v"(az), [nint] "+v"(nint), [ntr] "=&s"(ntr)           \
                : [tpx] "v"(tpx), [tpy] "v"(tpy), [tpz] "v"(tpz), [cN] "v"(cNg), [cY] "v"(cYg), [cS] "v"(cSg), [hT] "v"(hT),          \
-                 [trow] "v"(trow_a), [lane4] "v"(lane4), [tail] "s"(tail_q), [reach2] "s"(wp.reach2), [tiny] "s"(1e-290),           \
-                 [asmthfac] "s"(wp.asmthfac), [ec0] "s"(wp.ec[0]), [ec1] "s"(wp.ec[1]), [ec2] "s"(wp.ec[2]), [ec3] "s"(wp.ec[3]),   \
-                 [utor2wpi] "s"(wp.utor2wpi), [ym] "s"(wp.ym), [h2max] "s"(h2max), [etab] "s"(etab_a)                              \
+                 [trow] "v"(trow_a), [lane4] "v"(lane4), [tail] "s"(tail_q), [kc] "s"(kc), [etab] "v"(etab_a)                         \
                : ER_TRIP_CLOBBERS)
                       if constexpr(YUK)
-                        ER_TRIP_CALL(ER_TRIP4_ASM(ER_YUK_ET, ER_FST_OFF_ET));
+                        ER_TRIP_CALL(ER_TRIP4_ASM(ER_KC_TRIP_YUK, ER_YUK_ET, ER_FST_OFF_ET));
                       else
-                        ER_TRIP_CALL(ER_TRIP4_ASM(ER_NOYUK, ER_FST_OFF_NOET));
+                        ER_TRIP_CALL(ER_TRIP4_ASM(ER_KC_TRIP_NOYUK, ER_NOYUK, ER_FST_OFF_NOET));
 #undef ER_TRIP_CALL
                       st_iters += ntr;
                     }
@@ -437,17 +481,16 @@
                   if(!LW && usoft)
                     {
                       int cnt;
-#define ER_CULL_CALL(WRAPSEG)                                                                                                     \
-  asm volatile(ER_CULL_ASM(WRAPSEG)                                                                                                \
+#define ER_CULL_CALL(KCSEG, WRAPSEG)                                                                                              \
+  asm volatile(ER_CULL_ASM(KCSEG, WRAPSEG)                                                                                         \
                : [cnt] "=&s"(cnt)                                                                                                   \
                : [rx] "v"(rx), [ry] "v"(ry), [rz] "v"(rz), [rw] "v"(rw), [bcx] "s"(bcx), [bcy] "s"(bcy), [bcz] "s"(bcz), [bhx] "s"(bhx),  \
-                 [bhy] "s"(bhy), [bhz] "s"(bhz), [reach2] "s"(wp.reach2), [box] "s"(wp.box), [invbox] "s"(invbox), [wrpos] "s"(wr_pos),   \
-                 [q0] "s"(q0), [q1] "s"(q1), [q2] "s"(q2)                                                                           \
+                 [bhy] "s"(bhy), [bhz] "s"(bhz), [wrpos] "s"(wr_pos), [q0] "s"(q0), [q1] "s"(q1), [q2] "s"(q2), [kc] "s"(kc)              \
                : ER_CULL_CLOBBERS)
                       if(nowrap)
-                        ER_CULL_CALL("");
+                        ER_CULL_CALL(ER_KC_CULL, "");
                       else
-                        ER_CULL_CALL(ER_CULL_WRAP);
+                        ER_CULL_CALL(ER_KC_CULL_WRAP, ER_CULL_WRAP);
 #undef ER_CULL_CALL
                       wr_pos += cnt;
                     }
@@ -570,22 +613,25 @@
       else
         run_lists(std::false_type{});
 
+      ga = er_group_args();
       {
         int st_nodes = 0, st_batches = 0;
+        const int SG = ga->SG;
         if(grel % SG == 0)
           {
-            const long long u_cnt = (g_cnt + SG - 1) / SG;
-            st_nodes = __builtin_amdgcn_readfirstlane(gcount[NG * u_cnt + ru]);
-            st_batches = __builtin_amdgcn_readfirstlane(gcount[(NG + 1) * u_cnt + ru]);
+            const long long u_cnt = (ga->g_cnt + SG - 1) / SG;
+            st_nodes = __builtin_amdgcn_readfirstlane(ga->gcount[NG * u_cnt + ru]);
+            st_batches = __builtin_amdgcn_readfirstlane(ga->gcount[(NG + 1) * u_cnt + ru]);
           }
         acc_st[0] += (unsigned long long)st_entries;
         acc_st[1] += (unsigned long long)st_nodes;
         acc_st[2] += (unsigned long long)st_batches;
         acc_st[3] += (unsigned long long)st_iters;
       }
-      if(S > 1)
+      const int S_ = ga->S;
+      if(S_ > 1)
         {
-          for(int off = 1; off < S; off <<= 1)
+          for(int off = 1; off < S_; off <<= 1)
             {
               ax += __shfl_xor(ax, off);
               ay += __shfl_xor(ay, off);
@@ -593,23 +639,26 @@
               nint += __shfl_xor(nint, off);
             }
         }
-      if(valid && (lane & (S - 1)) == 0)
+      if(valid && (lane & (S_ - 1)) == 0)
         {
+          ER_GLOBAL double *const r_acc = ga->r_acc;
           r_acc[3 * ti + 0] = ax;
           r_acc[3 * ti + 1] = ay;
           r_acc[3 * ti + 2] = az;
-          r_nint[ti] = nint;
+          ga->r_nint[ti] = nint;
         }
     }
   if(lane == 0)
     {
-      unsigned long long *st64 = reinterpret_cast<unsigned long long *>(counter + 16);
+      unsigned long long *st64 = (unsigned long long *)(er_group_args()->counter + 16);
 #pragma unroll
       for(int qq = 0; qq < 4; qq++)
         if(acc_st[qq])
           atomicAdd(&st64[qq], acc_st[qq]);
     }
 }
+
+__global__ void k_set_eval_consts(EvalConsts v, EvalConsts *dst) { *dst = v; }
 
 static size_t er_fixed_bytes(const WalkParams &wp, bool yuk)
 {
@@ -638,10 +687,49 @@
   const size_t fixed = er_fixed_bytes(wp, YUK);
   const size_t lds = fixed + (size_t)waves * ((size_t)K * ER_SLOT);
   auto ke = k_eval_ring<NG, YUK, ET>;
+  EvalConsts kc;
+  memset(&kc, 0, sizeof(kc));
+  kc.reach2 = wp.reach2;
+  for(int q = 0; q < NGRAVS_NTYPES; q++)
+    kc.h2max = fmax(kc.h2max, wp.fsoft[q] * wp.fsoft[q]);
+  kc.asmthfac = wp.asmthfac;
+  kc.utor2wpi = wp.utor2wpi;
+  kc.ym = wp.ym;
+  for(int k = 0; k < 4; k++)
+    kc.ec[k] = wp.ec[k];
+  kc.tiny = 1e-290;
+  kc.box = wp.box;
+  kc.invbox = wp.box > 0 ? 1.0 / wp.box : 0.0;
+  if(!c->eval_consts.p || memcmp(&kc, &c->eval_consts_host, sizeof(kc)) != 0)
+    {
+      if(c->eval_consts.ensure(1))
+        return NGRAVS_ERR_NOMEM;
+      hipLaunchKernelGGL(k_set_eval_consts, dim3(1), dim3(1), 0, c->stream, kc, c->eval_consts.p);
+      c->eval_consts_host = kc;
+    }
   HIP_TRY(c, hipFuncSetAttribute(reinterpret_cast<const void *>(ke), hipFuncAttributeMaxDynamicSharedMemorySize, (int)lds));
-  hipLaunchKernelGGL(ke, dim3((unsigned)nblk), dim3(waves * 64), lds, c->stream, tv.mom, tv.flags, c->s_pm.p, c->s_type.p, c->s_active.p, c->table.p, wp,
-                     (long long)c->shard_first, t_count, c->walk_counters.p, c->r_acc.p, c->r_nint.p, region, gcount, g0, nb, lcap, scap,
-                     S, tlist, SG, K);
+  ErGroupArgs ga;
+  ga.t_first = (long long)c->shard_first;
+  ga.t_count = t_count;
+  ga.counter = (ER_GLOBAL int *)c->walk_counters.p;
+  ga.r_acc = (ER_GLOBAL double *)c->r_acc.p;
+  ga.r_nint = (ER_GLOBAL int *)c->r_nint.p;
+  ga.region_base = (const ER_GLOBAL int *)region;
+  ga.gcount = (const ER_GLOBAL int *)gcount;
+  ga.g_first = g0;
+  ga.g_cnt = nb;
+  ga.lcap = lcap;
+  ga.scap = scap;
+  ga.S = S;
+  ga.SG = SG;
+  ga.tlist = (const ER_GLOBAL int *)tlist;
+  ga.s_active = (const ER_GLOBAL unsigned char *)c->s_active.p;
+  ga.s_pm = (const ER_GLOBAL er_d4 *)c->s_pm.p;
+  ga.n_mom = (const ER_GLOBAL er_d4 *)tv.mom;
+  ga.s_type = (const ER_GLOBAL unsigned char *)c->s_type.p;
+  ga.n_flags = (const ER_GLOBAL int *)tv.flags;
+  ga.wp = wp;
+  hipLaunchKernelGGL(ke, dim3((unsigned)nblk), dim3(waves * 64), lds, c->stream, ga, c->table.p, c->eval_consts.p, K);
   return NGRAVS_OK;
 }
 
```
